# vlongle/pixie

Hardware: AMD Instinct MI355X
Metric: voxels/s (128^3 U-Net fwd) + MPM particle-steps/s (higher is better)
Workload: dtype f32 (operands split fp16 hi+lo, 3 f16 MFMAs/product, fp32 accumulate); 1 GPU; 128^3x64 feature grid -> SegmentationUNet+RegressionUNet forward (+argmax/one-hot combine), 1 scene per GPU per step; grid=128, feature_channels=64, parallelism=scene-parallel x1, executor=c+hip_graph

## Files before the change

### include/pixie_hip.h

```cpp
#ifndef PIXIE_HIP_H
#define PIXIE_HIP_H

#include <stdint.h>

#ifdef __cplusplus
extern "C" {
#endif

const char* pixie_last_error(void);
const char* pixie_build_arch(void);

typedef struct pixie_mpm pixie_mpm;

int pixie_mpm_create(pixie_mpm** out, int n_particles, int n_grid, double grid_lim);
int pixie_mpm_destroy(pixie_mpm* h);
int pixie_mpm_regrid(pixie_mpm* h, int n_grid, double grid_lim, void* stream);

int pixie_mpm_set_field(pixie_mpm* h, const char* name, const void* d_src, int64_t count, void* stream);
int pixie_mpm_get_field(pixie_mpm* h, const char* name, void* d_dst, int64_t count, void* stream);
int pixie_mpm_fill_field(pixie_mpm* h, const char* name, double value, void* stream);

int pixie_mpm_set_scalar(pixie_mpm* h, const char* key, double value);
int pixie_mpm_get_scalar(pixie_mpm* h, const char* key, double* value);

int pixie_mpm_update_mass(pixie_mpm* h, void* stream);
int pixie_mpm_finalize_mu_lam(pixie_mpm* h, int with_bulk, void* stream);
int pixie_mpm_apply_additional_params(pixie_mpm* h, const double point[3], const double size[3], double E,
                                      double nu, double density, int material, void* stream);
int pixie_mpm_apply_additional_params_batch(pixie_mpm* h, int64_t n_boxes, const float* d_boxes, const float* d_params,
                                            const int32_t* d_material, void* stream);

enum { PIXIE_BC_SURFACE = 0, PIXIE_BC_CUBOID = 1, PIXIE_BC_BBOX = 2 };
typedef struct pixie_bc_desc {
    int32_t type;
    int32_t surface_type;
    int32_t reset;
    int32_t pad_;
    double point[3], size[3], velocity[3], normal[3];
    double start_time, end_time, friction;
} pixie_bc_desc;
int pixie_mpm_add_bc(pixie_mpm* h, const pixie_bc_desc* bc);

enum { PIXIE_PM_IMPULSE = 0, PIXIE_PM_TRANSLATION = 1, PIXIE_PM_ROTATION = 2 };
typedef struct pixie_pmod_desc {
    int32_t type;
    int32_t pad_;
    double point[3], size[3];
    double force[3];
    double velocity[3];
    double normal[3], h1[3], h2[3];
    double half_height, radius, rotation_scale, translation_scale;
    double start_time, end_time;
} pixie_pmod_desc;
int pixie_mpm_add_particle_modifier(pixie_mpm* h, const pixie_pmod_desc* pm, void* stream);

int pixie_mpm_step(pixie_mpm* h, double dt, int n_substeps, void* stream);

typedef struct pixie_mpm_batch pixie_mpm_batch;
typedef struct pixie_batch_sched {
    double dt;
    int32_t steps_per_chunk;
    int32_t n_chunks;
    int32_t n_out;
    int32_t pad_;
    double shift[3], scale, mean[3];
    double inv_rotation[9];
    float* d_pos;
    float* d_cov;
} pixie_batch_sched;
int pixie_mpm_batch_create(pixie_mpm_batch** out, pixie_mpm* const* handles, int n_handles);
int pixie_mpm_batch_step(pixie_mpm_batch* b, double dt, int n_substeps, void* stream);
int pixie_mpm_batch_run(pixie_mpm_batch* b, const pixie_batch_sched* per_scene, int n_scenes, void* stream);
typedef struct pixie_batch_splat_out {
    float* d_log_scale;
    float* d_quat;
} pixie_batch_splat_out;
int pixie_mpm_batch_run_splats(pixie_mpm_batch* b, const pixie_batch_sched* per_scene, const pixie_batch_splat_out* splats ,
                               int n_scenes, void* stream);
int pixie_mpm_batch_destroy(pixie_mpm_batch* b);

int pixie_mpm_export_cov(pixie_mpm* h, float* d_cov , void* stream);
int pixie_mpm_export_R(pixie_mpm* h, float* d_R , void* stream);
int pixie_mpm_export_frame(pixie_mpm* h, int n_out, const double shift[3], double scale, const double mean[3],
                           const double inv_rotation[9], float* d_pos , float* d_cov ,
                           void* stream);
int pixie_splat_from_cov(const float* d_cov , int64_t n, float* d_log_scale , float* d_quat ,
                         void* stream);
int pixie_mpm_export_frame_splats(pixie_mpm* h, int n_out, const double shift[3], double scale, const double mean[3],
                                  const double inv_rotation[9], float* d_pos , float* d_cov ,
                                  float* d_log_scale , float* d_quat , void* stream);
int pixie_mpm_out_of_bounds(pixie_mpm* h, int64_t* count, void* stream);


typedef struct pixie_conv_desc {
    const float* d_in0; int32_t c0;
    const float* d_in1; int32_t c1;
    int32_t in_d, in_h, in_w;
    int32_t upsample;
    int32_t stride;
    int32_t ksize;
    const float* d_pro_a; const float* d_pro_b;
    const float* d_gamma; const float* d_beta;
    int32_t act;
    const float* d_w; const float* d_bias;
    int32_t c_out;
    const float* d_residual;
    float* d_out;
    const void* d_w16;
    const uint32_t* d_in_amax0; const uint32_t* d_in_amax1;
    float in_bound;
    float* d_out_stats;
    uint32_t* d_out_amax;
    void* d_workspace;
    int32_t out_d, out_h, out_w;
    const float* d_skip_in0; int32_t skip_c0;
    const float* d_skip_in1; int32_t skip_c1;
    const void* d_skip_w16; const float* d_skip_bias;
    const uint32_t* d_skip_amax0; const uint32_t* d_skip_amax1;
    int32_t w16_subpixel;
} pixie_conv_desc;

int pixie_conv_cout_padded(int c_out);
int pixie_conv_pack_weights(const float* d_w_oidhw, float* d_w_packed, int c_out, int c_in, int ksize, void* stream);
int64_t pixie_conv_packed16_bytes(int c_out, int c_in, int ksize);
int pixie_conv_pack_weights_f16x2(const float* d_w_oidhw, void* d_packed, int c_out, int c_in, int ksize, void* stream);
int64_t pixie_conv_subpixel_bytes(int c_out, int c_in);
int pixie_conv_pack_weights_subpixel(const float* d_w_oidhw, void* d_packed, int c_out, int c_in, void* stream);
int pixie_conv3d_forward(const pixie_conv_desc* desc, void* stream);
int64_t pixie_conv_stats_floats(const pixie_conv_desc* desc);
int64_t pixie_conv_workspace_bytes(const pixie_conv_desc* desc);
int pixie_stats_finalize(const float* d_stats, const pixie_conv_desc* desc, double* d_sums, void* stream);
int pixie_stats_norm_finalize(const float* d_stats0, const pixie_conv_desc* desc0, double* d_sums0, const float* d_stats1,
                              const pixie_conv_desc* desc1, double* d_sums1, int c1, int64_t spatial, int mode, int groups,
                              double eps, const float* d_weight, const float* d_bias, float* d_a, float* d_b, void* stream);
int pixie_conv_skip_foldable(const pixie_conv_desc* desc);

int pixie_channel_sums(const float* d_x, int channels, int64_t spatial, double* d_sums, void* stream);
int pixie_channel_stats(const float* d_x, int channels, int64_t spatial, double* d_sums, uint32_t* d_amax, void* stream);
int pixie_tensor_amax(const float* d_x, int64_t count, uint32_t* d_slot, void* stream);
int pixie_norm_finalize(const double* d_sums, int channels, int64_t spatial, int mode, int groups, double eps,
                        const float* d_weight, const float* d_bias, float* d_a, float* d_b, void* stream);

int pixie_attention_forward(const float* d_qkv, float* d_out, int channels, int tokens, void* stream);

int pixie_channel_affine(const float* d_x, const float* d_a, const float* d_b, float* d_y, int channels,
                         int64_t spatial, void* stream);

int pixie_voxel_grid_to_ncdhw(const void* d_feat_dhwc_f16, int d, int h, int w, int channels, float* d_out_cdhw, void* stream);

int pixie_projector_conv0(const void* d_feat_dhwc_f16, int64_t voxels, int channels, int n_networks, const void* const* d_w16,
                          const float* const* d_bias, float* const* d_out, int c_out, void* stream);

int pixie_pack_fields(const float* d_cont, const int32_t* d_seg_pred, int64_t n_scenes, int64_t spatial, void* d_wire, int64_t wire_bytes,
                      void* stream);

int pixie_combine_predictions(const float* d_logits, int num_classes, const float* d_cont, int64_t spatial,
                              float* d_combined, int32_t* d_argmax , void* stream);

int pixie_combine_class_ids(const int32_t* d_seg_pred, int num_classes, const float* d_cont, int64_t spatial, float* d_combined,
                            void* stream);

typedef struct pixie_unet pixie_unet;
typedef struct pixie_unet_config {
    int32_t feature_channels, cond_dim, model_channels, num_res_blocks;
    int32_t n_channel_mult; int32_t channel_mult[8];
    int32_t n_attention_resolutions; int32_t attention_resolutions[8];
    int32_t grid_size;
    int32_t out_channels;
    int32_t precision;
} pixie_unet_config;

int pixie_unet_create(pixie_unet** out, const pixie_unet_config* cfg);
int pixie_unet_destroy(pixie_unet* h);
int pixie_unet_param_count(const pixie_unet* h);
int pixie_unet_param_info(const pixie_unet* h, int index, const char** key, int64_t* numel, int32_t* ndim, int64_t shape[5]);
int pixie_unet_set_param(pixie_unet* h, const char* key, const float* d_values, int64_t numel);
int64_t pixie_unet_workspace_bytes(pixie_unet* h, int d, int hh, int w);
int pixie_unet_forward(pixie_unet* h, const float* d_feat, const float* d_proj0, int d, int hh, int w, float* d_out,
                       void* d_workspace, int64_t workspace_bytes, void* stream);
int pixie_unet_set_option(pixie_unet* h, const char* key, int value);

typedef struct pixie_field_desc {
    const float* d_pred;
    const uint8_t* d_mask;
    const float* d_axis_x; const float* d_axis_y; const float* d_axis_z;
    int32_t n_classes, d, h, w;
    double min_spacing;
    double density_min, density_max, E_min, E_max, nu_min, nu_max;
} pixie_field_desc;
int pixie_field_to_particles(const pixie_field_desc* field, const float* d_pos, int n, int k, double nn_distance_threshold,
                             int weighted, int default_material, int default_part_label, float* d_density, float* d_E,
                             float* d_nu, int32_t* d_material, int32_t* d_part_label, float* d_conf, float* d_nearest,
                             void* d_scratch, void* stream);

int pixie_unscale_prediction(const float* d_pred, int channels, int64_t spatial, double density_min, double density_max,
                             double E_min, double E_max, double nu_min, double nu_max, float* d_out, void* stream);
int64_t pixie_field_points_scratch_bytes(const pixie_field_desc* field);
int pixie_field_points(const pixie_field_desc* field, int64_t capacity, float* d_xyz , float* d_density, float* d_E,
                       float* d_nu, int32_t* d_material, float* d_conf, int64_t* d_count, void* d_scratch, void* stream);

int pixie_dbscan_roots(const float* d_pos_sorted, const int32_t* d_orig_index, const int32_t* d_cell_start, int n, int nx, int ny, int nz,
                       const double lo[3], double cell_size, double eps, int min_samples, int32_t* d_core_scratch,
                       int32_t* d_parent_scratch, int32_t* d_root, void* stream);

int pixie_fill_densify(const float* d_pos, const float* d_opacity, const float* d_cov6, int n, int grid_n, double grid_dx,
                       int32_t* d_grid_count, float* d_grid_density, void* stream);
int pixie_fill_dense_cells(int32_t* d_grid_count, const float* d_grid_density, int grid_n, double grid_dx, double density_thres,
                           int max_particles_per_cell, float* d_new_particles , int64_t max_samples,
                           uint64_t* d_counter, uint32_t seed, void* stream);
int pixie_fill_internal_cells(int32_t* d_grid_count, const float* d_grid_density, int grid_n, double grid_dx, int max_particles_per_cell,
                              int exclude_dir, int ray_cast_dir, double threshold, float* d_new_particles, int64_t max_samples,
                              uint64_t* d_counter, uint32_t seed, void* stream);
int pixie_particle_volume(const float* d_pos, int n, int grid_n, double grid_dx, int32_t* d_grid_count_scratch, float* d_vol, void* stream);
int pixie_nearest_particle(const float* d_pos, int n, const float* d_new_pos, int n_new, int32_t* d_nearest, void* stream);

typedef struct pixie_raster_desc {
    int32_t n, width, height;
    float tanfovx, tanfovy, scale_modifier;
    float viewmatrix[16], projmatrix[16], bg[3];
    int32_t pad_;
    const float* d_means;
    const float* d_cov3d;
    const float* d_scales;
    const float* d_rotations;
    const float* d_colors;
    const float* d_opacity;
    float* d_out_color;
    int32_t* d_radii;
    float* d_final_T;
    int32_t* d_n_contrib;
    void* d_workspace;
    int64_t workspace_bytes;
} pixie_raster_desc;
int64_t pixie_raster_workspace_bytes(int n, int width, int height, int64_t max_instances);
int pixie_raster_forward(const pixie_raster_desc* desc, int64_t* instances_out, void* stream);
int pixie_sh_to_rgb(const float* d_shs, int64_t n, int k_coeffs, int degree, const float* d_pos , const float campos[3],
                    const float* d_rot , int64_t n_rot, float* d_out , void* stream);

#ifdef PIXIE_DIAG
int pixie_mpm_phase(pixie_mpm* h, int phase, double dt, void* stream);

int pixie_mpm_kernel_times(pixie_mpm* h, double* particle_ms, double* grid_ms, int64_t* n_launches);

int pixie_conv_kernel_variant(const pixie_conv_desc* desc, int* slices);

int pixie_conv_tile_geometry(const pixie_conv_desc* desc, int32_t out[10]);
int pixie_conv_stats_layout(const pixie_conv_desc* desc, int64_t out[6]);
#endif

#ifdef __cplusplus
}
#endif
#endif
```

### pixie_amd/_lib.py

```python
from __future__ import annotations

import ctypes as C
import os

_HERE = os.path.dirname(os.path.abspath(__file__))
LIB_PATH = os.path.join(_HERE, "libpixie_hip.so")
DIAG_LIB_PATH = os.path.join(_HERE, "libpixie_hip_diag.so")


class PixieHipError(RuntimeError):
    pass


class BCDesc(C.Structure):
    _fields_ = [("type", C.c_int32), ("surface_type", C.c_int32), ("reset", C.c_int32), ("pad_", C.c_int32),
                ("point", C.c_double * 3), ("size", C.c_double * 3), ("velocity", C.c_double * 3),
                ("normal", C.c_double * 3), ("start_time", C.c_double), ("end_time", C.c_double),
                ("friction", C.c_double)]


class PModDesc(C.Structure):
    _fields_ = [("type", C.c_int32), ("pad_", C.c_int32),
                ("point", C.c_double * 3), ("size", C.c_double * 3), ("force", C.c_double * 3),
                ("velocity", C.c_double * 3), ("normal", C.c_double * 3), ("h1", C.c_double * 3),
                ("h2", C.c_double * 3), ("half_height", C.c_double), ("radius", C.c_double),
                ("rotation_scale", C.c_double), ("translation_scale", C.c_double),
                ("start_time", C.c_double), ("end_time", C.c_double)]


class ConvDesc(C.Structure):
    _fields_ = [("d_in0", C.c_void_p), ("c0", C.c_int32),
                ("d_in1", C.c_void_p), ("c1", C.c_int32),
                ("in_d", C.c_int32), ("in_h", C.c_int32), ("in_w", C.c_int32),
                ("upsample", C.c_int32), ("stride", C.c_int32), ("ksize", C.c_int32),
                ("d_pro_a", C.c_void_p), ("d_pro_b", C.c_void_p),
                ("d_gamma", C.c_void_p), ("d_beta", C.c_void_p),
                ("act", C.c_int32),
                ("d_w", C.c_void_p), ("d_bias", C.c_void_p),
                ("c_out", C.c_int32),
                ("d_residual", C.c_void_p), ("d_out", C.c_void_p),
                ("d_w16", C.c_void_p), ("d_in_amax0", C.c_void_p), ("d_in_amax1", C.c_void_p),
                ("in_bound", C.c_float),
                ("d_out_stats", C.c_void_p), ("d_out_amax", C.c_void_p),
                ("d_workspace", C.c_void_p),
                ("out_d", C.c_int32), ("out_h", C.c_int32), ("out_w", C.c_int32),
                ("d_skip_in0", C.c_void_p), ("skip_c0", C.c_int32),
                ("d_skip_in1", C.c_void_p), ("skip_c1", C.c_int32),
                ("d_skip_w16", C.c_void_p), ("d_skip_bias", C.c_void_p),
                ("d_skip_amax0", C.c_void_p), ("d_skip_amax1", C.c_void_p),
                ("w16_subpixel", C.c_int32)]


class UNetConfigC(C.Structure):
    _fields_ = [("feature_channels", C.c_int32), ("cond_dim", C.c_int32), ("model_channels", C.c_int32), ("num_res_blocks", C.c_int32),
                ("n_channel_mult", C.c_int32), ("channel_mult", C.c_int32 * 8),
                ("n_attention_resolutions", C.c_int32), ("attention_resolutions", C.c_int32 * 8),
                ("grid_size", C.c_int32), ("out_channels", C.c_int32), ("precision", C.c_int32)]


class BatchSched(C.Structure):
    _fields_ = [("dt", C.c_double), ("steps_per_chunk", C.c_int32), ("n_chunks", C.c_int32), ("n_out", C.c_int32), ("pad_", C.c_int32),
                ("shift", C.c_double * 3), ("scale", C.c_double), ("mean", C.c_double * 3), ("inv_rotation", C.c_double * 9),
                ("d_pos", C.c_void_p), ("d_cov", C.c_void_p)]


class BatchSplatOut(C.Structure):
    _fields_ = [("d_log_scale", C.c_void_p), ("d_quat", C.c_void_p)]


class FieldDesc(C.Structure):
    _fields_ = [("d_pred", C.c_void_p), ("d_mask", C.c_void_p),
                ("d_axis_x", C.c_void_p), ("d_axis_y", C.c_void_p), ("d_axis_z", C.c_void_p),
                ("n_classes", C.c_int32), ("d", C.c_int32), ("h", C.c_int32), ("w", C.c_int32),
                ("min_spacing", C.c_double),
                ("density_min", C.c_double), ("density_max", C.c_double), ("E_min", C.c_double), ("E_max", C.c_double),
                ("nu_min", C.c_double), ("nu_max", C.c_double)]


class RasterDesc(C.Structure):
    _fields_ = [("n", C.c_int32), ("width", C.c_int32), ("height", C.c_int32),
                ("tanfovx", C.c_float), ("tanfovy", C.c_float), ("scale_modifier", C.c_float),
                ("viewmatrix", C.c_float * 16), ("projmatrix", C.c_float * 16), ("bg", C.c_float * 3), ("pad_", C.c_int32),
                ("d_means", C.c_void_p), ("d_cov3d", C.c_void_p), ("d_scales", C.c_void_p), ("d_rotations", C.c_void_p),
                ("d_colors", C.c_void_p), ("d_opacity", C.c_void_p),
                ("d_out_color", C.c_void_p), ("d_radii", C.c_void_p), ("d_final_T", C.c_void_p), ("d_n_contrib", C.c_void_p),
                ("d_workspace", C.c_void_p), ("workspace_bytes", C.c_int64)]


_VP, _I, _I64, _D, _S = C.c_void_p, C.c_int, C.c_int64, C.c_double, C.c_char_p
_D3 = C.POINTER(C.c_double)
SIGNATURES = {
    "pixie_last_error": (C.c_char_p, []),
    "pixie_build_arch": (C.c_char_p, []),
    "pixie_mpm_create": (_I, [C.POINTER(_VP), _I, _I, _D]),
    "pixie_mpm_destroy": (_I, [_VP]),
    "pixie_mpm_regrid": (_I, [_VP, _I, _D, _VP]),
    "pixie_mpm_set_field": (_I, [_VP, _S, _VP, _I64, _VP]),
    "pixie_mpm_get_field": (_I, [_VP, _S, _VP, _I64, _VP]),
    "pixie_mpm_fill_field": (_I, [_VP, _S, _D, _VP]),
    "pixie_mpm_set_scalar": (_I, [_VP, _S, _D]),
    "pixie_mpm_get_scalar": (_I, [_VP, _S, C.POINTER(_D)]),
    "pixie_mpm_update_mass": (_I, [_VP, _VP]),
    "pixie_mpm_finalize_mu_lam": (_I, [_VP, _I, _VP]),
    "pixie_mpm_apply_additional_params": (_I, [_VP, _D3, _D3, _D, _D, _D, _I, _VP]),
    "pixie_mpm_apply_additional_params_batch": (_I, [_VP, _I64, _VP, _VP, _VP, _VP]),
    "pixie_mpm_add_bc": (_I, [_VP, C.POINTER(BCDesc)]),
    "pixie_mpm_add_particle_modifier": (_I, [_VP, C.POINTER(PModDesc), _VP]),
    "pixie_mpm_step": (_I, [_VP, _D, _I, _VP]),
    "pixie_mpm_export_cov": (_I, [_VP, _VP, _VP]),
    "pixie_mpm_export_R": (_I, [_VP, _VP, _VP]),
    "pixie_mpm_export_frame": (_I, [_VP, _I, _D3, _D, _D3, C.POINTER(C.c_double), _VP, _VP, _VP]),
    "pixie_mpm_out_of_bounds": (_I, [_VP, C.POINTER(_I64), _VP]),
    "pixie_mpm_batch_create": (_I, [C.POINTER(_VP), C.POINTER(_VP), _I]),
    "pixie_mpm_batch_step": (_I, [_VP, _D, _I, _VP]),
    "pixie_mpm_batch_run": (_I, [_VP, C.POINTER(BatchSched), _I, _VP]),
    "pixie_mpm_batch_run_splats": (_I, [_VP, C.POINTER(BatchSched), C.POINTER(BatchSplatOut), _I, _VP]),
    "pixie_splat_from_cov": (_I, [_VP, _I64, _VP, _VP, _VP]),
    "pixie_mpm_export_frame_splats": (_I, [_VP, _I, _D3, _D, _D3, C.POINTER(C.c_double), _VP, _VP, _VP, _VP, _VP]),
    "pixie_mpm_batch_destroy": (_I, [_VP]),
    "pixie_pack_fields": (_I, [_VP, _VP, _I64, _I64, _VP, _I64, _VP]),
    "pixie_conv_cout_padded": (_I, [_I]),
    "pixie_conv_pack_weights": (_I, [_VP, _VP, _I, _I, _I, _VP]),
    "pixie_conv_packed16_bytes": (_I64, [_I, _I, _I]),
    "pixie_conv_pack_weights_f16x2": (_I, [_VP, _VP, _I, _I, _I, _VP]),
    "pixie_conv_subpixel_bytes": (_I64, [_I, _I]),
    "pixie_conv_pack_weights_subpixel": (_I, [_VP, _VP, _I, _I, _VP]),
    "pixie_conv3d_forward": (_I, [C.POINTER(ConvDesc), _VP]),
    "pixie_conv_stats_floats": (_I64, [C.POINTER(ConvDesc)]),
    "pixie_conv_workspace_bytes": (_I64, [C.POINTER(ConvDesc)]),
    "pixie_stats_finalize": (_I, [_VP, C.POINTER(ConvDesc), _VP, _VP]),
    "pixie_stats_norm_finalize": (_I, [_VP, C.POINTER(ConvDesc), _VP, _VP, C.POINTER(ConvDesc), _VP, _I, _I64, _I, _I, _D, _VP, _VP, _VP, _VP, _VP]),
    "pixie_channel_stats": (_I, [_VP, _I, _I64, _VP, _VP, _VP]),
    "pixie_tensor_amax": (_I, [_VP, _I64, _VP, _VP]),
    "pixie_channel_sums": (_I, [_VP, _I, _I64, _VP, _VP]),
    "pixie_norm_finalize": (_I, [_VP, _I, _I64, _I, _I, _D, _VP, _VP, _VP, _VP, _VP]),
    "pixie_attention_forward": (_I, [_VP, _VP, _I, _I, _VP]),
    "pixie_channel_affine": (_I, [_VP, _VP, _VP, _VP, _I, _I64, _VP]),
    "pixie_projector_conv0": (_I, [_VP, _I64, _I, _I, C.POINTER(_VP), C.POINTER(_VP), C.POINTER(_VP), _I, _VP]),
    "pixie_conv_skip_foldable": (_I, [C.POINTER(ConvDesc)]),
    "pixie_unet_create": (_I, [C.POINTER(_VP), C.POINTER(UNetConfigC)]),
    "pixie_unet_destroy": (_I, [_VP]),
    "pixie_unet_param_count": (_I, [_VP]),
    "pixie_unet_param_info": (_I, [_VP, _I, C.POINTER(_S), C.POINTER(_I64), C.POINTER(C.c_int32), C.POINTER(_I64)]),
    "pixie_unet_set_param": (_I, [_VP, _S, _VP, _I64]),
    "pixie_unet_workspace_bytes": (_I64, [_VP, _I, _I, _I]),
    "pixie_unet_set_option": (_I, [_VP, _S, _I]),
    "pixie_unet_forward": (_I, [_VP, _VP, _VP, _I, _I, _I, _VP, _VP, _I64, _VP]),
    "pixie_combine_class_ids": (_I, [_VP, _I, _VP, _I64, _VP, _VP]),
    "pixie_combine_predictions": (_I, [_VP, _I, _VP, _I64, _VP, _VP, _VP]),
    "pixie_voxel_grid_to_ncdhw": (_I, [_VP, _I, _I, _I, _I, _VP, _VP]),
    "pixie_unscale_prediction": (_I, [_VP, _I, _I64, _D, _D, _D, _D, _D, _D, _VP, _VP]),
    "pixie_field_points_scratch_bytes": (_I64, [C.POINTER(FieldDesc)]),
    "pixie_field_points": (_I, [C.POINTER(FieldDesc), _I64, _VP, _VP, _VP, _VP, _VP, _VP, _VP, _VP, _VP]),
    "pixie_fill_densify": (_I, [_VP, _VP, _VP, _I, _I, _D, _VP, _VP, _VP]),
    "pixie_fill_dense_cells": (_I, [_VP, _VP, _I, _D, _D, _I, _VP, _I64, _VP, C.c_uint32, _VP]),
    "pixie_fill_internal_cells": (_I, [_VP, _VP, _I, _D, _I, _I, _I, _D, _VP, _I64, _VP, C.c_uint32, _VP]),
    "pixie_particle_volume": (_I, [_VP, _I, _I, _D, _VP, _VP, _VP]),
    "pixie_nearest_particle": (_I, [_VP, _I, _VP, _I, _VP, _VP]),
    "pixie_dbscan_roots": (_I, [_VP, _VP, _VP, _I, _I, _I, _I, C.POINTER(_D), _D, _D, _I, _VP, _VP, _VP, _VP]),
    "pixie_raster_workspace_bytes": (_I64, [_I, _I, _I, _I64]),
    "pixie_raster_forward": (_I, [C.POINTER(RasterDesc), C.POINTER(_I64), _VP]),
    "pixie_sh_to_rgb": (_I, [_VP, _I64, _I, _I, _VP, C.POINTER(C.c_float), _VP, _I64, _VP, _VP]),
    "pixie_field_to_particles": (_I, [C.POINTER(FieldDesc), _VP, _I, _I, _D, _I, _I, _I, _VP, _VP, _VP, _VP, _VP, _VP, _VP, _VP, _VP]),
}

DIAG_SIGNATURES = {
    "pixie_mpm_phase": (_I, [_VP, _I, _D, _VP]),
    "pixie_mpm_kernel_times": (_I, [_VP, C.POINTER(_D), C.POINTER(_D), C.POINTER(_I64)]),
    "pixie_conv_kernel_variant": (C.c_int, [C.POINTER(ConvDesc), C.POINTER(C.c_int)]),
    "pixie_conv_tile_geometry": (C.c_int, [C.POINTER(ConvDesc), C.POINTER(C.c_int32)]),
    "pixie_conv_stats_layout": (C.c_int, [C.POINTER(ConvDesc), C.POINTER(C.c_int64)]),
}

_libs = {}


def load(diag: bool = False):
    if diag in _libs:
        return _libs[diag]
    path = DIAG_LIB_PATH if diag else LIB_PATH
    if not os.path.exists(path):
        raise PixieHipError(
            f"{path} not found: build it with `python -m pixie_amd.build` (hipcc, gfx950). "
            "pixie_amd has no CPU fallback.")
    import torch
    lib = C.CDLL(path)
    for name, (res, args) in list(SIGNATURES.items()) + (list(DIAG_SIGNATURES.items()) if diag else []):
        fn = getattr(lib, name)
        fn.restype = res
        fn.argtypes = args
    _libs[diag] = lib
    return lib


def check(rc: int, what: str = "", lib=None):
    if rc != 0:
        msg = (lib or load()).pixie_last_error()
        raise PixieHipError(f"{what}: {msg.decode() if msg else 'unknown error'}")


def current_stream_ptr():
    import torch
    try:
        return C.c_void_p(torch._C._cuda_getCurrentRawStream(torch.cuda.current_device()))
    except AttributeError:
        return C.c_void_p(torch.cuda.current_stream().cuda_stream)


def d3(v):
    return (C.c_double * 3)(*[float(x) for x in v])
```

### pixie_amd/csrc/conv3d_f16x3.hip

```cpp
#include <hip/hip_runtime.h>

#include <cstdlib>
#include <map>
#include <string>
#include <type_traits>

#include "../../include/pixie_hip.h"
#include "common.h"
#include "conv_plan.h"

namespace pixie {

typedef float f32x16 __attribute__((ext_vector_type(16)));
typedef _Float16 f16x8 __attribute__((ext_vector_type(8)));

constexpr int kW16HeaderU4 = 4;

struct Conv16Args {
    const float* in0; const float* in1;
    int c0, cin;
    int ID, IH, IW;
    int LD, LH, LW;
    int ups;
    int stride;
// ... 786 lines not shown
    if (i < pairs)
        for (int pt = 0; pt < 64; ++pt) m = fmaxf(m, fabsf(subpixel_weight(src + i * 27, pt >> 3, pt & 7)));
    for (int off = 32; off > 0; off >>= 1) m = fmaxf(m, __shfl_down(m, off, 64));
    if ((threadIdx.x & 63) == 0 && m > 0.0f) atomicMax(slot, __float_as_uint(m));
}
__global__ void pack_weights_subpixel_kernel(const float* __restrict__ src, uint4* __restrict__ dst, int cout, int cin, int coutp,
                                             const unsigned* __restrict__ amax_bits) {
    const int KG = cin >> 3;
    const long total = 64L * KG * coutp;
    const long i = (long)blockIdx.x * blockDim.x + threadIdx.x;
    const int e = scale_exponent(__uint_as_float(*amax_bits));
    if (i == 0) dst[0] = make_uint4(__float_as_uint(pow2i(-e)), (unsigned)cout, (unsigned)cin, 64u);
    if (i >= total) return;
    const float s = pow2i(e);
    const int co = (int)(i % coutp);
    const long row = i / coutp;
    const int kg = (int)(row % KG);
    const int pt = (int)(row / KG);
    f16x8 vh, vl;
#pragma unroll
    for (int j = 0; j < 8; ++j) {
        float w = 0.0f;
        if (co < cout) w = subpixel_weight(src + ((long)co * cin + kg * 8 + j) * 27, pt >> 3, pt & 7) * s;
        const _Float16 h = (_Float16)w;
        vh[j] = h;
        vl[j] = (_Float16)(w - (float)h);
    }
    dst[kW16HeaderU4 + i] = __builtin_bit_cast(uint4, vh);
    dst[kW16HeaderU4 + total + i] = __builtin_bit_cast(uint4, vl);
}

static int reduce_segments(long osp) { return (int)((osp + kReduceSeg - 1) / kReduceSeg); }

bool conv_exact_v1() { return getenv("PIXIE_CONV_EXACT_V1") != nullptr; }

ConvShape conv_shape_of(const pixie_conv_desc* d) {
    ConvShape s;
    s.c0 = d->c0; s.c1 = d->c1; s.c_out = d->c_out;
    s.in_d = d->in_d; s.in_h = d->in_h; s.in_w = d->in_w;
    s.ksize = d->ksize; s.stride = d->stride; s.upsample = d->upsample;
    s.out_d = d->out_d; s.out_h = d->out_h; s.out_w = d->out_w;
    s.skip_c0 = d->skip_c0; s.skip_c1 = d->skip_c1;
    s.w16 = d->d_w16 != nullptr; s.subpixel = d->w16_subpixel != 0; s.workspace = d->d_workspace != nullptr; s.skip = d->d_skip_w16 != nullptr;
    s.exact_v1 = conv_exact_v1();
    return s;
}

static void conv_output_dims(const ConvShape& s, int& od, int& oh, int& ow) {
    const int pad = s.ksize == 3 ? 1 : 0;
    od = ((s.in_d << s.upsample) + 2 * pad - s.ksize) / s.stride + 1;
    oh = ((s.in_h << s.upsample) + 2 * pad - s.ksize) / s.stride + 1;
    ow = ((s.in_w << s.upsample) + 2 * pad - s.ksize) / s.stride + 1;
    if (s.out_d > 0) od = std::min(od, s.out_d);
    if (s.out_h > 0) oh = std::min(oh, s.out_h);
    if (s.out_w > 0) ow = std::min(ow, s.out_w);
}

ConvPlan conv_plan(const ConvShape& s) {
    ConvPlan p;
    auto refuse = [&p](ConvRefusal why) { p.path = CONV_NONE; p.refusal = why; return p; };
    if ((s.ksize != 1 && s.ksize != 3) || (s.stride != 1 && s.stride != 2) || (s.upsample != 0 && s.upsample != 1) || s.c0 <= 0 || s.c1 < 0 ||
        s.c_out <= 0 || s.in_d <= 0 || s.in_h <= 0 || s.in_w <= 0)
        return refuse(CONV_BAD_SHAPE);
    conv_output_dims(s, p.OD, p.OH, p.OW);
    p.KS = s.ksize; p.coutp = pixie_conv_cout_padded(s.c_out);
    p.ups = s.upsample; p.LD = s.in_d << p.ups; p.LH = s.in_h << p.ups; p.LW = s.in_w << p.ups;
    const int cin = s.c0 + s.c1;
    const bool stride_ok = s.stride == 1 || (s.ksize == 3 && !s.upsample), chunks_ok = cin % 16 == 0;
    if (!s.w16) {
        if (!stride_ok || !chunks_ok || s.exact_v1) { p.path = CONV_FIRST_GEN; return p; }
        p.path = CONV_EXACT_TILED;
    } else {
        if (!stride_ok) return refuse(CONV_BAD_STRIDE);
        if (!chunks_ok || s.c0 % 8 != 0) return refuse(CONV_BAD_CHANNELS);
        if (s.subpixel && !(s.upsample == 1 && s.ksize == 3 && s.stride == 1 && !s.skip)) return refuse(CONV_BAD_SUBPIXEL);
        p.path = s.subpixel ? CONV_F16X3_SUBPIXEL : CONV_F16X3;
    }
    const bool sub = p.path == CONV_F16X3_SUBPIXEL;
    const int chunks = cin / 16;
    const int smax = (p.f16x3() && s.workspace) ? std::min(8, chunks / 2) : 1;
    auto tile = [&p](int ED, int EH, int EW, int vox) {
        p.TX = pow2_le(EW, 32);
        p.TY = pow2_le(EH, std::max(1, std::min(4, vox / p.TX)));
        p.TZ = std::max(1, std::min(ED, vox / (p.TX * p.TY)));
        p.lTX = ilog2(p.TX); p.lTY = ilog2(p.TY);
        p.tiles_x = (EW + p.TX - 1) / p.TX; p.tiles_y = (EH + p.TY - 1) / p.TY; p.tiles_z = (ED + p.TZ - 1) / p.TZ;
        p.n_tiles = p.tiles_x * p.tiles_y * p.tiles_z;
    };
    if (sub) {
        p.ups = 0; p.LD = s.in_d; p.LH = s.in_h; p.LW = s.in_w;
        tile((p.OD + 1) / 2, (p.OH + 1) / 2, (p.OW + 1) / 2, 256);
        p.n_tiles *= 4;
        p.HX = p.TX + 2; p.HY = p.TY + 1; p.HZ = p.TZ + 1;
        p.MB = (p.coutp >= 64) ? 2 : 1; p.NB = 4;
        const long wgs = (long)p.n_tiles * ((p.coutp + p.MB * 32 - 1) / (p.MB * 32));
        while (p.slices * 2 <= smax && wgs * p.slices < 512) p.slices *= 2;
    } else {
        const long ovol = (long)p.OD * p.OH * p.OW;
        int MB = (p.coutp >= 64) ? 2 : 1;
        int NB = (s.stride == 2) ? 1 : 4;
        auto n_wg = [&](int mb, int nb) {
            const long tiles = (ovol + 128L * nb - 1) / (128L * nb);
            return tiles * ((p.coutp + mb * 32 - 1) / (mb * 32));
        };
        int slices = 1;
        if (smax >= 2 && n_wg(MB, NB) < 512) {
            bool found = false;
            for (int nb = NB; nb >= 1 && !found; nb /= 2) {
                for (int sl = 1; sl <= smax; sl *= 2)
                    if (n_wg(MB, nb) * sl >= 512) { NB = nb; slices = sl; found = true; break; }
            }
            if (!found) { NB = 1; slices = 1; while (slices * 2 <= smax) slices *= 2; }
        } else {
            while (n_wg(MB, NB) < 512 && NB > 1) NB /= 2;
            if (n_wg(MB, NB) < 512 && MB > 1) MB = 1;
        }
        p.MB = MB; p.NB = NB; p.slices = slices;
        tile(p.OD, p.OH, p.OW, 128 * NB);
        p.HX = (p.TX - 1) * s.stride + s.ksize; p.HY = (p.TY - 1) * s.stride + s.ksize; p.HZ = (p.TZ - 1) * s.stride + s.ksize;
    }
    p.HYX = p.HY * p.HX; p.CS = p.HZ * p.HYX;
    p.mHX = magic_of(p.HX); p.mHYX = magic_of(p.HYX);
    if (p.slices > 1) p.chunks_per_slice = (chunks + p.slices - 1) / p.slices;
    p.lds_bytes = (size_t)4 * p.CS * sizeof(uint4);
    if (p.lds_bytes > 160 * 1024) return refuse(CONV_BAD_LDS);
    const size_t epi_bytes = ((size_t)4 * 32 * (p.NB * 32 + 4) + (size_t)4 * p.MB * 32 * 2) * sizeof(float);
    if (p.slices == 1 && epi_bytes <= 80 * 1024) { p.epi_lds = 1; p.lds_bytes = std::max(p.lds_bytes, epi_bytes); }
    p.grid = dim3((unsigned)p.n_tiles, (unsigned)((p.coutp + p.MB * 32 - 1) / (p.MB * 32)), (unsigned)p.slices);
    if (!p.f16x3()) return p;
    const long osp = (long)p.OD * p.OH * p.OW;
    if (p.slices > 1) {
        const int n = reduce_segments(osp);
        p.stats = ConvStatLayout{n, n, 1, 1};
        p.stats_floats = (int64_t)s.c_out * n * 2 * (int64_t)(sizeof(double) / sizeof(float));
        p.workspace_bytes = (int64_t)p.slices * s.c_out * osp * (int64_t)sizeof(float);
    } else {
        p.stats = ConvStatLayout{p.n_tiles, 1, p.coutp, 0};
        p.stats_floats = (int64_t)p.n_tiles * p.coutp * 2;
    }
    p.fullres = !sub && p.slices == 1 && s.ksize == 3 && p.MB == 2 && p.NB == 4 && cin == 64 && s.c_out == 64 && s.stride == 1 && !s.upsample &&
                s.c1 == 0 && !s.skip && osp >= 128L * 128 * 128;
    const int scin = s.skip_c0 + s.skip_c1;
    p.skip_foldable = !sub && s.stride == 1 && !s.upsample && scin > 0 && scin % 16 == 0 && s.skip_c0 % 8 == 0 && p.slices == 1;
    return p;
}

using ConvKernel = void (*)(Conv16Args);
static ConvKernel conv16_kernel(const ConvPlan& p) {
    if (p.path == CONV_F16X3_SUBPIXEL) return p.MB == 2 ? conv3d_f16x3_subpixel_kernel<2> : conv3d_f16x3_subpixel_kernel<1>;
    if (p.fullres) return conv3d_f16x3_c64_fullres_kernel;
#define PX_CONV16_PICK(KS_, MB_, NB_) \
    if (p.KS == KS_ && p.MB == MB_ && p.NB == NB_) return p.path == CONV_EXACT_TILED ? conv3d_exact_kernel<KS_, MB_, NB_> : conv3d_f16x3_kernel<KS_, MB_, NB_>;
    PX_CONV_VARIANTS(PX_CONV16_PICK)
#undef PX_CONV16_PICK
    return nullptr;
}

static int launch(ConvKernel kern, const ConvPlan& p, const Conv16Args& a, hipStream_t st) {
    PX_REQUIRE(kern != nullptr, "conv: no kernel variant for ksize=%d MB=%d NB=%d", p.KS, p.MB, p.NB);
    PX_CHECK_HIP(allow_max_dynamic_lds(reinterpret_cast<const void*>(kern)));
    hipLaunchKernelGGL(kern, p.grid, dim3(256), p.lds_bytes, st, a);
    PX_CHECK_HIP(hipGetLastError());
    return 0;
}

static Conv16Args conv16_args(const pixie_conv_desc* d, const ConvPlan& p) {
    Conv16Args a{};
    a.in0 = d->d_in0; a.in1 = d->d_in1; a.c0 = d->c0; a.cin = d->c0 + d->c1;
    a.ID = d->in_d; a.IH = d->in_h; a.IW = d->in_w;
    a.LD = p.LD; a.LH = p.LH; a.LW = p.LW; a.ups = p.ups; a.stride = d->stride;
    a.OD = p.OD; a.OH = p.OH; a.OW = p.OW;
    a.pro_a = d->d_pro_a; a.pro_b = d->d_pro_b; a.gamma = d->d_gamma; a.beta = d->d_beta; a.act = d->act;
    a.bias = d->d_bias; a.cout = d->c_out; a.coutp = p.coutp;
    a.residual = d->d_residual; a.out = d->d_out;
    a.TX = p.TX; a.TY = p.TY; a.TZ = p.TZ; a.lTX = p.lTX; a.lTY = p.lTY;
    a.tiles_x = p.tiles_x; a.tiles_y = p.tiles_y; a.tiles_z = p.tiles_z; a.n_tiles = p.n_tiles;
    a.HX = p.HX; a.HY = p.HY; a.HZ = p.HZ; a.HYX = p.HYX; a.CS = p.CS; a.mHX = p.mHX; a.mHYX = p.mHYX;
    a.chunks_per_slice = p.chunks_per_slice; a.epi_lds = p.epi_lds;
    return a;
}

int conv3d_f16x3_forward(const pixie_conv_desc* d, const ConvPlan& p, hipStream_t st) {
    PX_REQUIRE(p.refusal != CONV_BAD_STRIDE, "f16x3 conv: stride must be 1, or 2 for a 3^3 kernel");
    PX_REQUIRE(p.refusal != CONV_BAD_CHANNELS, "f16x3 conv: c_in must be a multiple of 16 (got %d+%d)", d->c0, d->c1);
    PX_REQUIRE(d->d_in_amax0 != nullptr || d->in_bound > 0.0f, "f16x3 conv: needs d_in_amax0 or a positive in_bound");
    PX_REQUIRE(d->c1 == 0 || d->d_in_amax0 == nullptr || d->d_in_amax1 != nullptr, "f16x3 conv: second input needs its own amax slot");
    PX_REQUIRE(p.refusal != CONV_BAD_SUBPIXEL, "f16x3 conv: sub-pixel weights need upsample = 1, ksize = 3, stride = 1 and no folded skip");
    Conv16Args a = conv16_args(d, p);
    a.w16 = reinterpret_cast<const uint4*>(d->d_w16);
    a.amax0 = d->d_in_amax0; a.amax1 = (d->c1 > 0) ? d->d_in_amax1 : nullptr; a.in_bound = d->in_bound;
    a.stats = d->d_out_stats; a.out_amax = d->d_out_amax;
    if (d->d_skip_w16) {
        PX_REQUIRE(p.skip_foldable, "f16x3 conv: this launch cannot fold a skip convolution (pixie_conv_skip_foldable)");
        PX_REQUIRE(d->d_skip_in0 && d->d_skip_amax0 && (d->skip_c1 == 0 || (d->d_skip_in1 && d->d_skip_amax1)), "f16x3 conv: folded skip needs its inputs and their amax slots");
        a.sk_in0 = d->d_skip_in0; a.sk_in1 = d->d_skip_in1; a.sk_c0 = d->skip_c0; a.sk_cin = d->skip_c0 + d->skip_c1;
        a.sk_w16 = reinterpret_cast<const uint4*>(d->d_skip_w16); a.sk_bias = d->d_skip_bias;
        a.sk_amax0 = d->d_skip_amax0; a.sk_amax1 = d->skip_c1 > 0 ? d->d_skip_amax1 : nullptr;
    }
    if (p.slices > 1) {
        a.partial = static_cast<float*>(d->d_workspace);
        a.stats = nullptr; a.out_amax = nullptr;
    }
    PX_REQUIRE(p.refusal != CONV_BAD_LDS, "f16x3 conv: tile needs %zu B of LDS", p.lds_bytes);
    PX_REQUIRE(p.f16x3(), "f16x3 conv: bad sizes");
    if (int rc = launch(conv16_kernel(p), p, a, st)) return rc;
    if (p.slices == 1) return 0;
    const long osp = (long)a.OD * a.OH * a.OW, n_elems = (long)a.cout * osp;
    if (d->d_out_stats) {
        const dim3 rgrid((unsigned)reduce_segments(osp), (unsigned)a.cout);
        double* rstats = reinterpret_cast<double*>(d->d_out_stats);
        PX_REQUIRE((reinterpret_cast<size_t>(rstats) & 7) == 0, "f16x3 conv: d_out_stats of a split-K launch must be 8-byte aligned");
        const bool vec = osp % 4 == 0 && ((reinterpret_cast<size_t>(a.partial) | reinterpret_cast<size_t>(a.residual) | reinterpret_cast<size_t>(a.out)) & 15) == 0;
        if (vec) hipLaunchKernelGGL(splitk_reduce_stats_kernel<true>, rgrid, dim3(256), 0, st, a.partial, p.slices, n_elems, osp, a.bias, a.residual,
                                    a.out, rstats, d->d_out_amax);
        else hipLaunchKernelGGL(splitk_reduce_stats_kernel<false>, rgrid, dim3(256), 0, st, a.partial, p.slices, n_elems, osp, a.bias, a.residual,
                                a.out, rstats, d->d_out_amax);
    } else {
        hipLaunchKernelGGL(splitk_reduce_kernel, dim3((unsigned)((n_elems + 255) / 256)), dim3(256), 0, st, a.partial, p.slices, n_elems, osp,
                           a.bias, a.residual, a.out);
    }
    PX_CHECK_HIP(hipGetLastError());
    return 0;
}

int conv3d_exact_forward(const pixie_conv_desc* d, const ConvPlan& p, hipStream_t st) {
    PX_REQUIRE(p.refusal != CONV_BAD_LDS, "exact conv: tile needs %zu B of LDS", p.lds_bytes);
    PX_REQUIRE(p.path == CONV_EXACT_TILED, "exact conv: bad sizes");
    Conv16Args a = conv16_args(d, p);
    a.wf = d->d_w;
    a.in_bound = 1.0f;
    return launch(conv16_kernel(p), p, a, st);
}

}

using namespace pixie;

static ConvPlan plan_of(const pixie_conv_desc* d) { return d ? conv_plan(conv_shape_of(d)) : ConvPlan{}; }
static StatParts stat_parts(const ConvPlan& p, const void* stats) { return StatParts{stats, p.stats.n, p.stats.cstride, p.stats.tstride, p.stats.f64}; }

extern "C" int64_t pixie_conv_stats_floats(const pixie_conv_desc* d) { return plan_of(d).stats_floats; }

extern "C" int64_t pixie_conv_workspace_bytes(const pixie_conv_desc* d) {
    if (!d) return 0;
    ConvShape s = conv_shape_of(d);
    s.workspace = true;
    return conv_plan(s).workspace_bytes;
}

#ifdef PIXIE_DIAG
extern "C" int pixie_conv_kernel_variant(const pixie_conv_desc* d, int* slices_out) {
    const ConvPlan p = plan_of(d);
    if (slices_out) *slices_out = p.f16x3() ? p.slices : 1;
    if (!p.f16x3()) return 0;
    if (p.path == CONV_F16X3_SUBPIXEL) return 8300 + p.MB * 10 + p.NB;
    if (p.fullres) return 9324;
    return p.KS * 100 + p.MB * 10 + p.NB;
}

extern "C" int pixie_conv_tile_geometry(const pixie_conv_desc* d, int32_t out[10]) {
    const ConvPlan p = plan_of(d);
    if (!out || !p.tiled()) return 1;
    const int32_t v[10] = {p.TX, p.TY, p.TZ, p.tiles_x, p.tiles_y, p.tiles_z, p.epi_lds, p.slices, p.MB, p.NB};
    for (int i = 0; i < 10; ++i) out[i] = v[i];
    return 0;
}

extern "C" int pixie_conv_stats_layout(const pixie_conv_desc* d, int64_t out[6]) {
    const ConvPlan p = plan_of(d);
    if (!out || !p.f16x3()) return 1;
    out[0] = p.stats.n; out[1] = p.stats.cstride; out[2] = p.stats.tstride; out[3] = p.stats.f64; out[4] = p.stats.f64 ? kReduceSeg : 0;
    out[5] = p.coutp;
    return 0;
}
#endif

extern "C" int pixie_conv_skip_foldable(const pixie_conv_desc* d) { return plan_of(d).skip_foldable ? 1 : 0; }

extern "C" int pixie_stats_finalize(const float* d_stats, const pixie_conv_desc* d, double* d_sums, void* stream) {
    PX_REQUIRE(d_stats && d && d_sums, "pixie_stats_finalize: null argument");
    hipLaunchKernelGGL(stats_finalize_kernel, dim3((unsigned)d->c_out), dim3(256), 0, as_stream(stream), stat_parts(plan_of(d), d_stats), d_sums);
    PX_CHECK_HIP(hipGetLastError());
    return 0;
}

extern "C" int pixie_stats_norm_finalize(const float* d_stats0, const pixie_conv_desc* desc0, double* d_sums0, const float* d_stats1,
                                         const pixie_conv_desc* desc1, double* d_sums1, int c1, int64_t spatial, int mode, int groups,
                                         double eps, const float* d_weight, const float* d_bias, float* d_a, float* d_b, void* stream) {
    PX_REQUIRE(desc0 && d_sums0 && d_a && d_b && spatial > 0 && c1 >= 0, "pixie_stats_norm_finalize: bad arguments");
    PX_REQUIRE(c1 == 0 || d_sums1, "pixie_stats_norm_finalize: a second part needs d_sums1");
    PX_REQUIRE(!d_stats1 || desc1, "pixie_stats_norm_finalize: d_stats1 needs its descriptor");
    const int c0 = desc0->c_out, channels = c0 + c1;
    PX_REQUIRE(!d_stats1 || desc1->c_out == c1, "pixie_stats_norm_finalize: desc1 has %d output channels, c1 is %d", desc1 ? desc1->c_out : 0, c1);
    PX_REQUIRE(mode == 0 || (mode == 1 && groups > 0 && channels % groups == 0), "pixie_stats_norm_finalize: bad mode/groups");
    const StatParts none{nullptr, 0, 0, 0, 0};
    const StatParts p0 = d_stats0 ? stat_parts(plan_of(desc0), d_stats0) : none;
    const StatParts p1 = d_stats1 ? stat_parts(plan_of(desc1), d_stats1) : none;
    hipLaunchKernelGGL(stats_norm_finalize_kernel, dim3((unsigned)(mode == 0 ? channels : groups)), dim3(256), 0, as_stream(stream), p0, d_sums0, c0,
                       p1, d_sums1, channels, (double)spatial, mode, groups, eps, d_weight, d_bias, d_a, d_b);
    PX_CHECK_HIP(hipGetLastError());
    return 0;
}

extern "C" int64_t pixie_conv_packed16_bytes(int c_out, int c_in, int ksize) {
    if (c_out <= 0 || c_in <= 0 || c_in % 8 != 0 || (ksize != 1 && ksize != 3)) return 0;
    const int64_t taps = (int64_t)ksize * ksize * ksize;
    return ((int64_t)kW16HeaderU4 + 2 * taps * (c_in / 8) * pixie_conv_cout_padded(c_out)) * (int64_t)sizeof(uint4);
}

extern "C" int pixie_tensor_amax(const float* d_x, int64_t count, uint32_t* d_slot, void* stream) {
    PX_REQUIRE(d_x && d_slot && count > 0, "pixie_tensor_amax: bad arguments");
    const int blocks = (int)std::min<int64_t>(2048, (count + 1023) / 1024);
    hipLaunchKernelGGL(amax_kernel, dim3(blocks), dim3(256), 0, as_stream(stream), d_x, (long)count, d_slot);
    PX_CHECK_HIP(hipGetLastError());
    return 0;
}

extern "C" int pixie_conv_pack_weights_f16x2(const float* d_w, void* d_packed, int c_out, int c_in, int ksize, void* stream) {
    PX_REQUIRE(d_w && d_packed && c_out > 0 && c_in > 0 && c_in % 8 == 0 && (ksize == 1 || ksize == 3),
               "pixie_conv_pack_weights_f16x2: bad arguments (c_in must be a multiple of 8)");
    hipStream_t st = as_stream(stream);
    const int taps = ksize * ksize * ksize;
    const int coutp = pixie_conv_cout_padded(c_out);
    unsigned* slot = reinterpret_cast<unsigned*>(d_packed) + 15;
    PX_CHECK_HIP(hipMemsetAsync(d_packed, 0, kW16HeaderU4 * sizeof(uint4), st));
    if (pixie_tensor_amax(d_w, (int64_t)c_out * c_in * taps, slot, stream)) return 1;
    const long total = (long)taps * (c_in / 8) * coutp;
    hipLaunchKernelGGL(pack_weights_f16x2_kernel, dim3(cdiv(total, 256)), dim3(256), 0, st, d_w, reinterpret_cast<uint4*>(d_packed), c_out,
                       c_in, taps, coutp, slot);
    PX_CHECK_HIP(hipGetLastError());
    return 0;
}

extern "C" int64_t pixie_conv_subpixel_bytes(int c_out, int c_in) {
    if (c_out <= 0 || c_in <= 0 || c_in % 16 != 0) return 0;
    return ((int64_t)kW16HeaderU4 + 2 * 64 * (int64_t)(c_in / 8) * pixie_conv_cout_padded(c_out)) * (int64_t)sizeof(uint4);
}

extern "C" int pixie_conv_pack_weights_subpixel(const float* d_w, void* d_packed, int c_out, int c_in, void* stream) {
    PX_REQUIRE(d_w && d_packed && c_out > 0 && c_in > 0 && c_in % 16 == 0,
               "pixie_conv_pack_weights_subpixel: bad arguments (c_in must be a multiple of 16)");
    hipStream_t st = as_stream(stream);
    const int coutp = pixie_conv_cout_padded(c_out);
    unsigned* slot = reinterpret_cast<unsigned*>(d_packed) + 15;
    PX_CHECK_HIP(hipMemsetAsync(d_packed, 0, kW16HeaderU4 * sizeof(uint4), st));
    const long pairs = (long)c_out * c_in;
    hipLaunchKernelGGL(subpixel_amax_kernel, dim3(cdiv(pairs, 256)), dim3(256), 0, st, d_w, pairs, slot);
    PX_CHECK_HIP(hipGetLastError());
    const long total = 64L * (c_in / 8) * coutp;
    hipLaunchKernelGGL(pack_weights_subpixel_kernel, dim3(cdiv(total, 256)), dim3(256), 0, st, d_w, reinterpret_cast<uint4*>(d_packed), c_out,
                       c_in, coutp, slot);
    PX_CHECK_HIP(hipGetLastError());
    return 0;
}
```

### pixie_amd/csrc/projector_fused.hip

```cpp
#include <hip/hip_runtime.h>

#include "../../include/pixie_hip.h"
#include "common.h"

namespace pixie {

typedef float f32x16 __attribute__((ext_vector_type(16)));
typedef _Float16 f16x8 __attribute__((ext_vector_type(8)));

constexpr int kPW16HeaderU4 = 4;
constexpr int kPMaxNets = 2;
constexpr int kPKC = 64;

struct ProjArgs {
    const uint4* feat;
    long voxels;
    int C, KG;
    int nets, coutp, cout;
    const uint4* w16[kPMaxNets];
    const float* bias[kPMaxNets];
    float* out[kPMaxNets];
    int waves_m, nv;
};

__global__ __launch_bounds__(256, 2) void projector_conv0_kernel(ProjArgs A) {
    extern __shared__ uint4 xs[];
    const int tid = threadIdx.x, lane = tid & 63, wave = tid >> 6;
    const int kh = lane >> 5, l31 = lane & 31;
    const int wm = wave % A.waves_m, wn = wave / A.waves_m;
    const int row0 = wm * 64;
    const int net = row0 / A.coutp, co0 = row0 % A.coutp;
    const long v0 = (long)blockIdx.x * A.nv;
    const int vw = wn * 64;
    const int stride = A.nv + 1;

    f32x16 acc[2][2];
#pragma unroll
    for (int mb = 0; mb < 2; ++mb)
#pragma unroll
        for (int nb = 0; nb < 2; ++nb)
#pragma unroll
            for (int r = 0; r < 16; ++r) acc[mb][nb][r] = 0.0f;

    const uint4* wHi = A.w16[net] + kPW16HeaderU4 + co0 + l31;
    const size_t lo_off = (size_t)A.KG * A.coutp;
    const int units = A.nv * 8;

    for (int c_base = 0; c_base < A.C; c_base += kPKC) {
        __syncthreads();
        for (int u = tid; u < units; u += 256) {
            const int vox = u >> 3, kg = u & 7;
            const long v = v0 + vox;
            uint4 q = make_uint4(0u, 0u, 0u, 0u);
            if (v < A.voxels && c_base + 8 * kg < A.C) q = A.feat[v * A.KG + (c_base >> 3) + kg];
            xs[kg * stride + vox] = q;
        }
        __syncthreads();
#pragma unroll
        for (int ks = 0; ks < kPKC / 16; ++ks) {
            const int kg = (c_base >> 3) + 2 * ks + kh;
            if (c_base + 16 * ks >= A.C) break;
            f16x8 ah[2], al[2], b[2];
#pragma unroll
            for (int mb = 0; mb < 2; ++mb) {
                const uint4 h = wHi[(size_t)kg * A.coutp + mb * 32];
                const uint4 l = wHi[lo_off + (size_t)kg * A.coutp + mb * 32];
                ah[mb] = __builtin_bit_cast(f16x8, h);
                al[mb] = __builtin_bit_cast(f16x8, l);
            }
#pragma unroll
            for (int nb = 0; nb < 2; ++nb) b[nb] = __builtin_bit_cast(f16x8, xs[(2 * ks + kh) * stride + vw + nb * 32 + l31]);
#pragma unroll
            for (int mb = 0; mb < 2; ++mb)
#pragma unroll
                for (int nb = 0; nb < 2; ++nb) acc[mb][nb] = __builtin_amdgcn_mfma_f32_32x32x16_f16(al[mb], b[nb], acc[mb][nb], 0, 0, 0);
#pragma unroll
            for (int mb = 0; mb < 2; ++mb)
#pragma unroll
                for (int nb = 0; nb < 2; ++nb) acc[mb][nb] = __builtin_amdgcn_mfma_f32_32x32x16_f16(ah[mb], b[nb], acc[mb][nb], 0, 0, 0);
        }
    }

    const float inv = __uint_as_float(A.w16[net][0].x);
    float* out = A.out[net];
    const float* bias = A.bias[net];
#pragma unroll
    for (int mb = 0; mb < 2; ++mb)
#pragma unroll
        for (int r = 0; r < 16; ++r) {
            const int co = co0 + mb * 32 + (r & 3) + 8 * (r >> 2) + 4 * kh;
            if (co >= A.cout) continue;
            const float bv = bias ? bias[co] : 0.0f;
#pragma unroll
            for (int nb = 0; nb < 2; ++nb) {
                const long v = v0 + vw + nb * 32 + l31;
                if (v < A.voxels) out[(size_t)co * A.voxels + v] = acc[mb][nb][r] * inv + bv;
            }
        }
}

}

using namespace pixie;

extern "C" int pixie_projector_conv0(const void* d_feat_dhwc_f16, int64_t voxels, int channels, int n_networks, const void* const* d_w16,
                                     const float* const* d_bias, float* const* d_out, int c_out, void* stream) {
    PX_REQUIRE(d_feat_dhwc_f16 && d_w16 && d_out && voxels > 0, "pixie_projector_conv0: null argument");
    PX_REQUIRE(n_networks >= 1 && n_networks <= kPMaxNets, "pixie_projector_conv0: 1 or 2 networks");
    PX_REQUIRE(channels > 0 && channels % 16 == 0, "pixie_projector_conv0: the channel count must be a multiple of 16 (got %d)", channels);
    const int coutp = pixie_conv_cout_padded(c_out);
    PX_REQUIRE(c_out > 0 && coutp % 64 == 0, "pixie_projector_conv0: c_out must pad to a multiple of 64 (got %d -> %d)", c_out, coutp);
    const int rows = n_networks * coutp;
    PX_REQUIRE(rows == 64 || rows == 128 || rows == 256, "pixie_projector_conv0: %d x %d output rows are not a tiling this kernel has", n_networks, coutp);
    ProjArgs a{};
    a.feat = static_cast<const uint4*>(d_feat_dhwc_f16);
    a.voxels = voxels; a.C = channels; a.KG = channels / 8;
    a.nets = n_networks; a.coutp = coutp; a.cout = c_out;
    for (int n = 0; n < n_networks; ++n) {
        PX_REQUIRE(d_w16[n] && d_out[n], "pixie_projector_conv0: null weights / output for network %d", n);
        a.w16[n] = static_cast<const uint4*>(d_w16[n]);
        a.bias[n] = d_bias ? d_bias[n] : nullptr;
        a.out[n] = d_out[n];
    }
    a.waves_m = rows / 64;
    a.nv = (4 / a.waves_m) * 64;
    const size_t lds = (size_t)8 * (a.nv + 1) * sizeof(uint4);
    const long tiles = (voxels + a.nv - 1) / a.nv;
    hipLaunchKernelGGL(projector_conv0_kernel, dim3((unsigned)tiles), dim3(256), lds, as_stream(stream), a);
    PX_CHECK_HIP(hipGetLastError());
    return 0;
}
```

### pixie_amd/csrc/unet_exec.hip

```cpp
#include <hip/hip_runtime.h>

#include <algorithm>
#include <cmath>
#include <cstdlib>
#include <cstring>
#include <map>
#include <memory>
#include <stdexcept>
#include <string>
#include <tuple>
#include <unordered_map>
#include <vector>

#include "../../include/pixie_hip.h"
#include "common.h"
#include "conv_plan.h"

namespace pixie {
int channel_stats_prezeroed(const float* d_x, int channels, int64_t spatial, double* d_sums, uint32_t* d_amax, hipStream_t st);
int norm_finalize_cat(const double* d_sums0, int c0, const double* d_sums1, int c1, int64_t spatial, int mode, int groups, double eps,
                      const float* d_weight, const float* d_bias, float* d_a, float* d_b, hipStream_t st);
namespace {

enum { ACT_NONE = 0, ACT_LEAKY = 1, ACT_SILU = 2 };
enum Kind { CONV_IN, RES, DOWN, ATTN, UP };

struct Blk { Kind kind; std::string prefix; int cin, cout, sp; };
struct Plan {
    std::vector<std::vector<Blk>> in_blocks, out_blocks;
    std::vector<Blk> middle;
    int out_sp = 0;
};

struct Err : std::runtime_error { using std::runtime_error::runtime_error; };
[[noreturn]] void fail(const char* fmt, ...) {
    char buf[512];
    va_list ap; va_start(ap, fmt); vsnprintf(buf, sizeof buf, fmt, ap); va_end(ap);
    throw Err(buf);
}
void ok(int rc, const char* what) { if (rc != 0) fail("%s: %s", what, pixie_last_error()); }

bool has(const std::vector<int>& v, int x) { for (int e : v) if (e == x) return true; return false; }

struct Cfg {
    int feature_channels, cond_dim, model_channels, num_res_blocks;
    std::vector<int> mult, attn;
    int grid_size, out_channels, precision;
    bool has_projector() const { return feature_channels != cond_dim; }
    int projector_hidden() const { return feature_channels > cond_dim ? 128 : 0; }
};

Plan build_plan(const Cfg& c) {
    Plan p;
    const int mc = c.model_channels, nrb = c.num_res_blocks;
    auto name = [](const char* part, int idx, int sub) { return std::string("unet.") + part + "." + std::to_string(idx) + "." + std::to_string(sub); };
    p.in_blocks.push_back({Blk{CONV_IN, "unet.input_blocks.0.0", c.cond_dim, mc, c.grid_size}});
    std::vector<int> chans{mc}, sizes{c.grid_size};
    int ch = mc, ds = 1, sp = c.grid_size;
    for (size_t level = 0; level < c.mult.size(); ++level) {
        const int m = c.mult[level];
        for (int r = 0; r < nrb; ++r) {
            const int idx = (int)p.in_blocks.size();
            std::vector<Blk> seq{Blk{RES, name("input_blocks", idx, 0), ch, m * mc, sp}};
            ch = m * mc;
            if (has(c.attn, ds)) seq.push_back(Blk{ATTN, name("input_blocks", idx, 1), ch, ch, sp});
            p.in_blocks.push_back(seq);
            chans.push_back(ch);
        }
        if (level + 1 != c.mult.size()) {
            const int idx = (int)p.in_blocks.size();
            p.in_blocks.push_back({Blk{DOWN, name("input_blocks", idx, 0), ch, ch, sp}});
            chans.push_back(ch);
            sizes.push_back(sp);
            ds *= 2;
            sp = (sp + 1) / 2;
        }
    }
    p.middle = {Blk{RES, "unet.middle_block.0", ch, ch, sp}, Blk{ATTN, "unet.middle_block.1", ch, ch, sp}, Blk{RES, "unet.middle_block.2", ch, ch, sp}};
    for (int level = (int)c.mult.size() - 1; level >= 0; --level) {
        const int m = c.mult[level];
        for (int i = 0; i <= nrb; ++i) {
            const int idx = (int)p.out_blocks.size();
            const int ich = chans.back(); chans.pop_back();
            std::vector<Blk> seq{Blk{RES, name("output_blocks", idx, 0), ch + ich, mc * m, sp}};
            ch = mc * m;
            if (has(c.attn, ds)) seq.push_back(Blk{ATTN, name("output_blocks", idx, (int)seq.size()), ch, ch, sp});
            if (level && i == nrb) {
                seq.push_back(Blk{UP, name("output_blocks", idx, (int)seq.size()), ch, ch, sp});
                ds /= 2;
                sp = sizes.back(); sizes.pop_back();
            }
            p.out_blocks.push_back(seq);
        }
    }
    p.out_sp = sp;
    return p;
}

struct Param {
    std::string key;
    std::vector<int64_t> shape;
    int64_t numel = 1;
    bool norm = false;
    const float* d = nullptr;
    uint64_t version = 0;
};

std::vector<Param> param_table(const Cfg& c, const Plan& plan) {
    std::vector<Param> out;
    auto add = [&](const std::string& key, std::vector<int64_t> shape, bool norm) {
        Param p; p.key = key; p.shape = shape; p.norm = norm;
        for (int64_t s : shape) p.numel *= s;
        out.push_back(p);
    };
    auto conv = [&](const std::string& prefix, int cout, int cin, int k, int dims = 3) {
        std::vector<int64_t> s{cout, cin};
        for (int i = 0; i < dims; ++i) s.push_back(k);
        add(prefix + ".weight", s, false);
        add(prefix + ".bias", {cout}, false);
    };
    auto norm = [&](const std::string& prefix, std::vector<int64_t> shape) {
        add(prefix + ".weight", shape, true);
        add(prefix + ".bias", shape, true);
    };
    if (c.has_projector()) {
        const int hid = c.projector_hidden();
        if (!hid) {
            conv("projector.net.0", c.cond_dim, c.feature_channels, 1);
            norm("projector.net.1", {c.cond_dim});
        } else {
            conv("projector.net.0", hid, c.feature_channels, 1);
            norm("projector.net.1", {hid});
            conv("projector.net.3", hid, hid, 3);
            norm("projector.net.4", {hid});
            conv("projector.net.6", c.cond_dim, hid, 1);
            norm("projector.net.7", {c.cond_dim});
        }
    }
    auto emit = [&](const Blk& b) {
        const std::vector<int64_t> vol{b.sp, b.sp, b.sp};
        switch (b.kind) {
            case CONV_IN: conv(b.prefix, b.cout, b.cin, 3); break;
            case RES:
                norm(b.prefix + ".in_layers.0", vol);
                conv(b.prefix + ".in_layers.2", b.cout, b.cin, 3);
                norm(b.prefix + ".out_layers.0", vol);
                conv(b.prefix + ".out_layers.3", b.cout, b.cout, 3);
                if (b.cin != b.cout) conv(b.prefix + ".skip_connection", b.cout, b.cin, 1);
                break;
            case DOWN: conv(b.prefix + ".op", b.cout, b.cin, 3); break;
            case UP:   conv(b.prefix + ".conv", b.cout, b.cin, 3); break;
            case ATTN:
                norm(b.prefix + ".norm", {b.cin});
                conv(b.prefix + ".qkv", 3 * b.cin, b.cin, 1, 1);
                conv(b.prefix + ".proj_out", b.cin, b.cin, 1, 1);
                break;
        }
    };
    for (auto& seq : plan.in_blocks) for (auto& b : seq) emit(b);
    for (auto& b : plan.middle) emit(b);
    for (auto& seq : plan.out_blocks) for (auto& b : seq) emit(b);
    norm("unet.out.0", {plan.out_sp, plan.out_sp, plan.out_sp});
    conv("unet.out.2", c.out_channels, c.model_channels, 3);
    return out;
}

struct Arena {
    static constexpr int64_t kAlign = 256;
    char* base = nullptr;
    int64_t capacity = 0, peak = 0;
    std::map<int64_t, int64_t> free_;
    std::map<int64_t, int64_t> used_;

    void reset(char* b, int64_t cap) {
        base = b; capacity = cap; peak = 0;
        free_.clear(); used_.clear();
        free_[0] = cap;
    }
    int64_t alloc(int64_t bytes) {
        bytes = (bytes + kAlign - 1) / kAlign * kAlign;
        if (bytes == 0) bytes = kAlign;
        for (auto it = free_.begin(); it != free_.end(); ++it) {
            if (it->second < bytes) continue;
            const int64_t off = it->first, rest = it->second - bytes;
            free_.erase(it);
            if (rest > 0) free_[off + bytes] = rest;
            used_[off] = bytes;
            if (off + bytes > peak) peak = off + bytes;
            return off;
        }
        fail("pixie_unet_forward: the workspace is too small (%lld bytes; ask pixie_unet_workspace_bytes for this grid size)", (long long)capacity);
    }
    void release(int64_t off) {
        auto u = used_.find(off);
        if (u == used_.end()) return;
        int64_t size = u->second;
        used_.erase(u);
        auto next = free_.lower_bound(off);
        if (next != free_.end() && off + size == next->first) { size += next->second; next = free_.erase(next); }
        if (next != free_.begin()) {
            auto prev = std::prev(next);
            if (prev->first + prev->second == off) { prev->second += size; return; }
        }
        free_[off] = size;
    }
    template <class T> T* ptr(int64_t off) const { return reinterpret_cast<T*>(base + off); }
};

struct Exec;
struct Tens {
    Exec* ex = nullptr;
    float* p = nullptr;
    int64_t off = -1;
    int c = 0, d = 0, h = 0, w = 0;
    int64_t sums_off = -1;
    bool has_sums = false;
    double* sums = nullptr;
    int64_t partials_off = -1;
    pixie_conv_desc pdesc;
    uint32_t* slot = nullptr;
    int64_t spatial() const { return (int64_t)d * h * w; }
    ~Tens();
};
using TP = std::shared_ptr<Tens>;

struct Packed { void* d = nullptr; uint64_t version = ~0ull; };
struct Sized { int64_t bytes; int slots; int64_t zsum_doubles; };
struct Bound { float wmax = 0, bmax = 0; uint64_t wver = ~0ull, bver = ~0ull; };

}
}

using namespace pixie;

struct pixie_unet {
    Cfg cfg;
    Plan plan;
    std::vector<Param> params;
    std::unordered_map<std::string, int> index;
    std::unordered_map<std::string, Packed> packed32, packed16;
    std::unordered_map<std::string, Bound> bounds;
    uint32_t* d_bound_slots = nullptr;
    std::vector<uint32_t> h_bound_slots;
    std::map<std::tuple<int, int, int, bool>, Sized> sized;
    bool fuse_stats = true, split_k = true, fold_skip = true, subpixel = true;
    bool split_stats = true;
    struct Replay { const float* feat; const float* proj0; float* out; void* ws; int d; uint64_t epoch; hipGraph_t graph; hipGraphExec_t exec; };
    bool use_graph = false;
    uint64_t epoch = 0;
    std::vector<Replay> replays;
    static constexpr size_t kMaxReplays = 4;
    void drop_replay(size_t i) {
        (void)hipGraphExecDestroy(replays[i].exec);
        (void)hipGraphDestroy(replays[i].graph);
        replays.erase(replays.begin() + (long)i);
    }

    const Param& param(const std::string& key) const {
        auto it = index.find(key);
        if (it == index.end()) fail("pixie_unet: no parameter named '%s'", key.c_str());
        return params[it->second];
    }
};

namespace pixie {
namespace {

struct Exec {
    pixie_unet* net = nullptr;
    Arena arena;
    bool dry = false;
    void* stream = nullptr;
    uint32_t* slots = nullptr;
    int slot_next = 0, slot_cap = 0;
    double* zsums = nullptr;
    int64_t zsum_next = 0, zsum_cap = 0;

    TP make(int c, int d, int h, int w) {
        auto t = std::make_shared<Tens>();
        t->ex = this; t->c = c; t->d = d; t->h = h; t->w = w;
        t->off = arena.alloc((int64_t)c * d * h * w * sizeof(float));
        t->p = arena.ptr<float>(t->off);
        return t;
    }
    TP external(const float* p, int c, int d, int h, int w) {
        auto t = std::make_shared<Tens>();
        t->ex = this; t->p = const_cast<float*>(p); t->c = c; t->d = d; t->h = h; t->w = w;
        return t;
    }
    uint32_t* new_slot() {
        if (!dry && slot_next >= slot_cap) fail("pixie_unet_forward: out of |x|max slots (internal sizing error)");
        return dry ? (slot_next++, nullptr) : slots + slot_next++;
    }
    struct Scratch {
        Exec* ex; int64_t off;
        Scratch(Exec* e, int64_t bytes) : ex(e), off(e->arena.alloc(bytes)) {}
        ~Scratch() { ex->arena.release(off); }
        template <class T> T* as() const { return ex->arena.ptr<T>(off); }
    };

    const float* P(const std::string& key) {
        const Param& p = net->param(key);
        if (!dry && !p.d) fail("pixie_unet_forward: parameter '%s' was never set", key.c_str());
        return p.d;
    }
    const void* w16(const std::string& key, bool subpixel = false) {
        const Param& p = net->param(key + ".weight");
        if (dry) return nullptr;
        Packed& e = net->packed16[subpixel ? key + "#subpixel" : key];
        if (e.version != p.version) {
            const int cout = (int)p.shape[0], cin = (int)p.shape[1], k = (int)p.shape[2];
            const int64_t nb = subpixel ? (k == 3 ? pixie_conv_subpixel_bytes(cout, cin) : 0) : pixie_conv_packed16_bytes(cout, cin, k);
            if (nb <= 0) fail("pixie_unet: '%s' cannot take the f16x3 packing (c_in %d)", key.c_str(), cin);
            if (!e.d && hipMalloc(&e.d, (size_t)nb) != hipSuccess) fail("pixie_unet: hipMalloc of %lld bytes failed", (long long)nb);
            if (!p.d) fail("pixie_unet_forward: parameter '%s.weight' was never set", key.c_str());
            if (subpixel) ok(pixie_conv_pack_weights_subpixel(p.d, e.d, cout, cin, stream), "pixie_conv_pack_weights_subpixel");
            else ok(pixie_conv_pack_weights_f16x2(p.d, e.d, cout, cin, k, stream), "pixie_conv_pack_weights_f16x2");
            e.version = p.version;
        }
        return e.d;
    }
    const float* w32(const std::string& key) {
        const Param& p = net->param(key + ".weight");
        if (dry) return nullptr;
        Packed& e = net->packed32[key];
        if (e.version != p.version) {
            const int cout = (int)p.shape[0], cin = (int)p.shape[1], k = (int)p.shape[2];
            int64_t taps = 1;
            for (size_t i = 2; i < p.shape.size(); ++i) taps *= p.shape[i];
            const int64_t nb = taps * cin * pixie_conv_cout_padded(cout) * (int64_t)sizeof(float);
            if (!e.d && hipMalloc(&e.d, (size_t)nb) != hipSuccess) fail("pixie_unet: hipMalloc of %lld bytes failed", (long long)nb);
            if (!p.d) fail("pixie_unet_forward: parameter '%s.weight' was never set", key.c_str());
            ok(pixie_conv_pack_weights(p.d, static_cast<float*>(e.d), cout, cin, k, stream), "pixie_conv_pack_weights");
            e.version = p.version;
        }
        return static_cast<const float*>(e.d);
    }
    float norm_bound(const std::string& key, int64_t count) {
        if (dry) return 1.0f;
        const Bound& b = net->bounds[key];
        return (float)(std::sqrt((double)count) * (double)b.wmax + (double)b.bmax + 1e-30);
    }

    void stats(const TP& t) {
        if (t->has_sums || t->partials_off >= 0) return;
        t->has_sums = true;
        if (!dry && zsum_next + 2 * t->c > zsum_cap) fail("pixie_unet_forward: out of statistics space (internal sizing error)");
        t->sums = dry ? nullptr : zsums + zsum_next;
        zsum_next += 2 * t->c;
        t->slot = new_slot();
        if (!dry) ok(channel_stats_prezeroed(t->p, t->c, t->spatial(), t->sums, t->slot, as_stream(stream)), "pixie_channel_stats");
    }
    struct AB { std::shared_ptr<Scratch> mem; float* a; float* b; };
    AB norm_finalize(const std::vector<TP>& parts, int64_t spatial, int mode, int groups, const float* w, const float* b) {
        for (auto& t : parts) stats(t);
        const Tens* t0 = parts[0].get();
        const Tens* t1 = parts.size() > 1 ? parts[1].get() : nullptr;
        const int c0 = t0->c, c1 = t1 ? t1->c : 0, c = c0 + c1;
        AB r;
        const int cpad = (c + 63) / 64 * 64;
        r.mem = std::make_shared<Scratch>(this, (int64_t)(cpad + c) * sizeof(float));
        r.a = r.mem->as<float>();
        r.b = r.a + cpad;
        const bool p0 = t0->partials_off >= 0, p1 = t1 && t1->partials_off >= 0;
        if (p0 || p1) {
            pixie_conv_desc d0 = t0->pdesc;
            if (!p0) { std::memset(&d0, 0, sizeof d0); d0.c_out = c0; }
            if (!dry) ok(pixie_stats_norm_finalize(p0 ? arena.ptr<float>(t0->partials_off) : nullptr, &d0, t0->sums,
                                                   p1 ? arena.ptr<float>(t1->partials_off) : nullptr, p1 ? &t1->pdesc : nullptr, t1 ? t1->sums : nullptr,
                                                   c1, spatial, mode, groups, 1e-5, w, b, r.a, r.b, stream), "pixie_stats_norm_finalize");
            for (auto& t : parts)
                if (t->partials_off >= 0) { arena.release(t->partials_off); t->partials_off = -1; t->has_sums = true; }
        } else if (!t1) {
            if (!dry) ok(pixie_norm_finalize(t0->sums, c, spatial, mode, groups, 1e-5, w, b, r.a, r.b, stream), "pixie_norm_finalize");
        } else {
            if (!dry) ok(norm_finalize_cat(t0->sums, c0, t1->sums, c1, spatial, mode, groups, 1e-5, w, b, r.a, r.b, as_stream(stream)), "pixie_norm_finalize");
        }
        return r;
    }

    ConvPlan plan_conv(ConvShape& s, const std::vector<TP>& parts, int cout, int ksize, int stride, bool upsample) const {
        s.c0 = parts[0]->c; s.c1 = parts.size() > 1 ? parts[1]->c : 0; s.c_out = cout;
        s.in_d = parts[0]->d; s.in_h = parts[0]->h; s.in_w = parts[0]->w;
        s.ksize = ksize; s.stride = stride; s.upsample = upsample ? 1 : 0;
        s.w16 = net->cfg.precision == 0; s.workspace = net->split_k; s.exact_v1 = conv_exact_v1();
        ConvPlan p = conv_plan(s);
        if (p.refusal == CONV_BAD_CHANNELS) { s.w16 = s.subpixel = s.skip = false; p = conv_plan(s); }
        return p;
    }
    bool skip_foldable(const TP& x, int cout, int ksize, const std::vector<TP>& sp) const {
        ConvShape s;
        s.skip_c0 = sp[0]->c; s.skip_c1 = sp.size() > 1 ? sp[1]->c : 0;
        return plan_conv(s, {x}, cout, ksize, 1, false).skip_foldable;
    }

    struct ConvOpt {
        int stride = 1; bool upsample = false;
        const AB* pro = nullptr; std::string affine_store;
        int act = ACT_NONE; TP residual; float bound = 0.0f;
        int out_d = 0, out_h = 0, out_w = 0;
        float* out_ptr = nullptr;
        const std::vector<TP>* skip_parts = nullptr; std::string skip_key;
    };
    TP conv(const std::vector<TP>& parts, const std::string& wkey, int cout, int ksize, const ConvOpt& o) {
        const TP& x0 = parts[0];
        const Tens* x1 = parts.size() > 1 ? parts[1].get() : nullptr;
        ConvShape s;
        s.out_d = o.out_d; s.out_h = o.out_h; s.out_w = o.out_w;
        s.subpixel = net->subpixel && o.upsample && ksize == 3 && o.stride == 1;
        if (o.skip_parts) { s.skip = true; s.skip_c0 = (*o.skip_parts)[0]->c; s.skip_c1 = o.skip_parts->size() > 1 ? (*o.skip_parts)[1]->c : 0; }
        const ConvPlan plan = plan_conv(s, parts, cout, ksize, o.stride, o.upsample);
        const int od = plan.OD, oh = plan.OH, ow = plan.OW;
        pixie_conv_desc desc;
        std::memset(&desc, 0, sizeof desc);
        if (o.out_d) { desc.out_d = od; desc.out_h = oh; desc.out_w = ow; }
        const bool f16 = s.w16;
        const bool raw = !o.pro && o.affine_store.empty();
        if (f16 && raw) for (auto& t : parts) stats(t);

        TP out = o.out_ptr ? external(o.out_ptr, cout, od, oh, ow) : make(cout, od, oh, ow);
        desc.d_in0 = x0->p; desc.c0 = x0->c;
        desc.d_in1 = x1 ? x1->p : nullptr; desc.c1 = x1 ? x1->c : 0;
        desc.in_d = x0->d; desc.in_h = x0->h; desc.in_w = x0->w;
        desc.upsample = o.upsample ? 1 : 0;
        desc.stride = o.stride;
        desc.ksize = ksize;
        if (o.pro) { desc.d_pro_a = o.pro->a; desc.d_pro_b = o.pro->b; }
        if (!o.affine_store.empty()) { desc.d_gamma = P(o.affine_store + ".weight"); desc.d_beta = P(o.affine_store + ".bias"); }
        desc.act = o.act;
        desc.d_bias = P(wkey + ".bias");
        desc.c_out = cout;
        desc.d_residual = o.residual ? o.residual->p : nullptr;
        desc.d_out = out->p;
        if (!f16) {
            desc.d_w = w32(wkey);
            if (!dry) ok(pixie_conv3d_forward(&desc, stream), "pixie_conv3d_forward");
            return out;
        }
        desc.d_w16 = w16(wkey, s.subpixel);
        desc.w16_subpixel = s.subpixel ? 1 : 0;
        if (o.skip_parts) {
            const std::vector<TP>& sp = *o.skip_parts;
            desc.d_skip_in0 = sp[0]->p; desc.skip_c0 = sp[0]->c;
            desc.d_skip_in1 = sp.size() > 1 ? sp[1]->p : nullptr; desc.skip_c1 = sp.size() > 1 ? sp[1]->c : 0;
            desc.d_skip_w16 = w16(o.skip_key);
            desc.d_skip_bias = P(o.skip_key + ".bias");
            desc.d_skip_amax0 = sp[0]->slot; desc.d_skip_amax1 = sp.size() > 1 ? sp[1]->slot : nullptr;
        }
        if (raw) {
            desc.d_in_amax0 = parts[0]->slot;
            desc.d_in_amax1 = x1 ? parts[1]->slot : nullptr;
        } else {
            desc.in_bound = o.bound;
        }
        std::unique_ptr<Scratch> workspace;
        if (plan.workspace_bytes > 0) { workspace.reset(new Scratch(this, plan.workspace_bytes)); desc.d_workspace = workspace->as<void>(); }
        bool have_stats = false;
        if (net->fuse_stats) {
            uint32_t* slot = new_slot();
            const int64_t nfl = plan.stats_floats;
            if (nfl > 0 && (!workspace || net->split_stats)) {
                out->partials_off = arena.alloc(nfl * (int64_t)sizeof(float));
                desc.d_out_stats = arena.ptr<float>(out->partials_off);
                desc.d_out_amax = slot;
                have_stats = true;
                out->slot = slot;
            }
        }
        if (!dry) ok(pixie_conv3d_forward(&desc, stream), "pixie_conv3d_forward");
        if (have_stats) {
            out->sums_off = arena.alloc((int64_t)cout * 2 * sizeof(double));
            out->sums = arena.ptr<double>(out->sums_off);
            out->pdesc = desc;
        }
        return out;
    }

    TP res(const Blk& b, const std::vector<TP>& parts) {
        const std::string& p = b.prefix;
        const int64_t spatial = parts[0]->spatial();
        AB pro = norm_finalize(parts, spatial, 0, 1, nullptr, nullptr);
        ConvOpt o1; o1.pro = &pro; o1.affine_store = p + ".in_layers.0"; o1.act = ACT_LEAKY; o1.bound = norm_bound(p + ".in_layers.0", spatial);
        TP h = conv(parts, p + ".in_layers.2", b.cout, 3, o1);
        AB pro2 = norm_finalize({h}, spatial, 0, 1, nullptr, nullptr);
        TP skip = parts[0];
        ConvOpt o2; o2.pro = &pro2; o2.affine_store = p + ".out_layers.0"; o2.act = ACT_LEAKY; o2.bound = norm_bound(p + ".out_layers.0", spatial);
        if (b.cin != b.cout) {
            if (net->fold_skip && skip_foldable(h, b.cout, 3, parts)) {
                skip.reset();
                for (auto& t : parts) stats(t);
                o2.skip_parts = &parts; o2.skip_key = p + ".skip_connection";
            } else {
                skip = conv(parts, p + ".skip_connection", b.cout, 1, ConvOpt{});
            }
        }
        o2.residual = skip;
        return conv({h}, p + ".out_layers.3", b.cout, 3, o2);
    }
    TP attn(const Blk& b, const TP& x) {
        const std::string& p = b.prefix;
        const int c = x->c;
        const int64_t spatial = x->spatial();
        AB pro = norm_finalize({x}, spatial, 1, 32, P(p + ".norm.weight"), P(p + ".norm.bias"));
        ConvOpt o; o.pro = &pro; o.bound = norm_bound(p + ".norm", spatial * (c / 32));
        TP qkv = conv({x}, p + ".qkv", 3 * c, 1, o);
        TP att = make(c, x->d, x->h, x->w);
        if (!dry) ok(pixie_attention_forward(qkv->p, att->p, c, (int)spatial, stream), "pixie_attention_forward");
        qkv.reset();
        ConvOpt o2; o2.residual = x;
        return conv({att}, p + ".proj_out", c, 1, o2);
    }
    TP block(const Blk& b, const std::vector<TP>& parts, const Tens* up_to) {
        if (b.kind == RES) return res(b, parts);
        const TP& x = parts[0];
        if (b.kind == ATTN) return attn(b, x);
        if (b.kind == DOWN) { ConvOpt o; o.stride = 2; return conv({x}, b.prefix + ".op", b.cout, 3, o); }
        if (b.kind == UP) {
            ConvOpt o; o.upsample = true;
            if (up_to) { o.out_d = up_to->d; o.out_h = up_to->h; o.out_w = up_to->w; }
            return conv({x}, b.prefix + ".conv", b.cout, 3, o);
        }
        fail("pixie_unet: unexpected block kind");
    }

    TP forward(const float* d_feat, const float* d_proj0, int D, int H, int W, float* d_out) {
        const Cfg& c = net->cfg;
        const int64_t spatial = (int64_t)D * H * W;
        TP x;
        AB pro_in; const AB* pro_in_p = nullptr;
        int act_in = ACT_NONE; float bound_in = 0.0f;
        if (c.has_projector()) {
            const std::string q = "projector.net.";
            const int hid = c.projector_hidden();
            if (!hid) {
                const int g = std::max(c.cond_dim / 2, 1);
                x = conv({external(d_feat, c.feature_channels, D, H, W)}, q + "0", c.cond_dim, 1, ConvOpt{});
                pro_in = norm_finalize({x}, spatial, 1, g, P(q + "1.weight"), P(q + "1.bias"));
                act_in = ACT_SILU;
                bound_in = norm_bound(q + "1", spatial * (c.cond_dim / g));
            } else {
                if (d_proj0) x = external(d_proj0, hid, D, H, W);
                else x = conv({external(d_feat, c.feature_channels, D, H, W)}, q + "0", hid, 1, ConvOpt{});
                AB pro = norm_finalize({x}, spatial, 1, 32, P(q + "1.weight"), P(q + "1.bias"));
                ConvOpt o; o.pro = &pro; o.act = ACT_SILU; o.bound = norm_bound(q + "1", spatial * (hid / 32));
                x = conv({x}, q + "3", hid, 3, o);
                AB pro2 = norm_finalize({x}, spatial, 1, 32, P(q + "4.weight"), P(q + "4.bias"));
                ConvOpt o2; o2.pro = &pro2; o2.act = ACT_SILU; o2.bound = norm_bound(q + "4", spatial * (hid / 32));
                x = conv({x}, q + "6", c.cond_dim, 1, o2);
                pro_in = norm_finalize({x}, spatial, 1, 32, P(q + "7.weight"), P(q + "7.bias"));
                bound_in = norm_bound(q + "7", spatial * std::max(c.cond_dim / 32, 1));
            }
            pro_in_p = &pro_in;
        } else {
            x = external(d_feat, c.feature_channels, D, H, W);
        }
        const Plan& plan = net->plan;
        std::vector<TP> hs;
        const Blk& first = plan.in_blocks[0][0];
        ConvOpt of; of.pro = pro_in_p; of.act = act_in; of.bound = bound_in;
        TP h = conv({x}, first.prefix, first.cout, 3, of);
        x.reset();
        pro_in = AB{};
        hs.push_back(h);
        for (size_t i = 1; i < plan.in_blocks.size(); ++i) {
            for (const Blk& b : plan.in_blocks[i]) h = block(b, {h}, nullptr);
            hs.push_back(h);
        }
        for (const Blk& b : plan.middle) h = block(b, {h}, nullptr);
        for (auto& seq : plan.out_blocks) {
            TP skip = hs.back(); hs.pop_back();
            if (skip->d != h->d || skip->h != h->h || skip->w != h->w) fail("pixie_unet_forward: skip tensor and decoder tensor differ in size");
            std::vector<TP> parts{h, skip};
            h.reset(); skip.reset();
            for (const Blk& b : seq) {
                TP nh = block(b, parts, (b.kind == UP && !hs.empty()) ? hs.back().get() : nullptr);
                parts.clear();
                parts.push_back(nh);
            }
            h = parts[0];
        }
        AB pro = norm_finalize({h}, h->spatial(), 0, 1, nullptr, nullptr);
        ConvOpt oo; oo.pro = &pro; oo.affine_store = "unet.out.0"; oo.act = ACT_LEAKY; oo.bound = norm_bound("unet.out.0", h->spatial());
        oo.out_ptr = d_out;
        return conv({h}, "unet.out.2", c.out_channels, 3, oo);
    }
};

Tens::~Tens() {
    if (!ex) return;
    if (off >= 0) ex->arena.release(off);
    if (sums_off >= 0) ex->arena.release(sums_off);
    if (partials_off >= 0) ex->arena.release(partials_off);
}

void refresh_bounds(pixie_unet* net, void* stream) {
    std::vector<std::pair<std::string, int>> todo;
    int n_norm = 0;
    for (const Param& p : net->params) {
        if (!p.norm || p.key.size() < 7 || p.key.compare(p.key.size() - 7, 7, ".weight") != 0) continue;
        const std::string key = p.key.substr(0, p.key.size() - 7);
        const Param& pb = net->param(key + ".bias");
        Bound& b = net->bounds[key];
        if (b.wver != p.version || b.bver != pb.version) todo.push_back({key, 2 * n_norm});
        ++n_norm;
    }
    if (todo.empty()) return;
    const size_t bytes = (size_t)2 * n_norm * sizeof(uint32_t);
    if (!net->d_bound_slots && hipMalloc(&net->d_bound_slots, bytes) != hipSuccess) fail("pixie_unet: hipMalloc failed");
    net->h_bound_slots.assign((size_t)2 * n_norm, 0u);
    hipStream_t s = as_stream(stream);
    if (hipMemsetAsync(net->d_bound_slots, 0, bytes, s) != hipSuccess) fail("pixie_unet: hipMemsetAsync failed");
    for (auto& t : todo) {
        const Param& pw = net->param(t.first + ".weight");
        const Param& pb = net->param(t.first + ".bias");
        if (!pw.d || !pb.d) fail("pixie_unet_forward: parameter '%s' was never set", t.first.c_str());
        ok(pixie_tensor_amax(pw.d, pw.numel, net->d_bound_slots + t.second, stream), "pixie_tensor_amax");
        ok(pixie_tensor_amax(pb.d, pb.numel, net->d_bound_slots + t.second + 1, stream), "pixie_tensor_amax");
    }
    if (hipMemcpyAsync(net->h_bound_slots.data(), net->d_bound_slots, bytes, hipMemcpyDeviceToHost, s) != hipSuccess ||
        hipStreamSynchronize(s) != hipSuccess)
        fail("pixie_unet: reading the normalisation bounds back failed: %s", hipGetErrorString(hipGetLastError()));
    for (auto& t : todo) {
        Bound& b = net->bounds[t.first];
        std::memcpy(&b.wmax, &net->h_bound_slots[t.second], 4);
        std::memcpy(&b.bmax, &net->h_bound_slots[t.second + 1], 4);
        b.wver = net->param(t.first + ".weight").version;
        b.bver = net->param(t.first + ".bias").version;
    }
}

__global__ void zero_head_kernel(uint4* p, int64_t n16) {
    const int64_t i = (int64_t)blockIdx.x * 256 + threadIdx.x;
    if (i < n16) p[i] = make_uint4(0u, 0u, 0u, 0u);
}

constexpr int64_t kSlotAlign = 256;
int64_t slot_region_bytes(int n_slots) { return ((int64_t)n_slots * 4 + kSlotAlign - 1) / kSlotAlign * kSlotAlign; }
int64_t zsum_region_bytes(int64_t n_doubles) { return (n_doubles * 8 + kSlotAlign - 1) / kSlotAlign * kSlotAlign; }

Sized size_pass(pixie_unet* net, int D, int H, int W, bool from_proj0) {
    auto key = std::make_tuple(D, H, W, from_proj0);
    auto it = net->sized.find(key);
    if (it != net->sized.end()) return it->second;
    Exec ex;
    ex.net = net; ex.dry = true; ex.stream = nullptr;
    ex.arena.reset(reinterpret_cast<char*>(0x10000000), (int64_t)1 << 50);
    {
        const float* fake = reinterpret_cast<const float*>(0x100);
        TP out = ex.forward(from_proj0 ? nullptr : fake, from_proj0 ? fake : nullptr, D, H, W, reinterpret_cast<float*>(0x100));
    }
    Sized r{ex.arena.peak + slot_region_bytes(ex.slot_next) + zsum_region_bytes(ex.zsum_next), ex.slot_next, ex.zsum_next};
    net->sized[key] = r;
    return r;
}

template <class F> int guarded(F f) {
    try { return f(); }
    catch (const std::exception& e) { return set_error("%s", e.what()); }
}

}
}

extern "C" int pixie_unet_create(pixie_unet** out, const pixie_unet_config* c) {
    PX_REQUIRE(out && c, "pixie_unet_create: null argument");
    PX_REQUIRE(c->n_channel_mult >= 1 && c->n_channel_mult <= 8 && c->n_attention_resolutions >= 0 && c->n_attention_resolutions <= 8,
               "pixie_unet_create: channel_mult needs 1..8 entries, attention_resolutions 0..8");
    PX_REQUIRE(c->feature_channels > 0 && c->cond_dim > 0 && c->model_channels > 0 && c->num_res_blocks > 0 && c->grid_size > 0 && c->out_channels > 0,
               "pixie_unet_create: non-positive size");
    PX_REQUIRE(c->precision == 0 || c->precision == 1, "pixie_unet_create: precision is 0 (f16x3) or 1 (exact fp32)");
    return guarded([&] {
        std::unique_ptr<pixie_unet> n(new pixie_unet);
        n->cfg.feature_channels = c->feature_channels; n->cfg.cond_dim = c->cond_dim; n->cfg.model_channels = c->model_channels;
        n->cfg.num_res_blocks = c->num_res_blocks; n->cfg.grid_size = c->grid_size; n->cfg.out_channels = c->out_channels;
        n->cfg.precision = c->precision;
        n->cfg.mult.assign(c->channel_mult, c->channel_mult + c->n_channel_mult);
        n->cfg.attn.assign(c->attention_resolutions, c->attention_resolutions + c->n_attention_resolutions);
        n->plan = build_plan(n->cfg);
        n->params = param_table(n->cfg, n->plan);
        for (size_t i = 0; i < n->params.size(); ++i) n->index[n->params[i].key] = (int)i;
        const char* fs = getenv("PIXIE_FUSE_STATS"); n->fuse_stats = !(fs && fs[0] == '0');
        const char* sk = getenv("PIXIE_CONV_SPLIT_K"); n->split_k = !(sk && sk[0] == '0');
        const char* fk = getenv("PIXIE_FOLD_SKIP"); n->fold_skip = !(fk && fk[0] == '0');
        const char* ss = getenv("PIXIE_SPLIT_STATS"); n->split_stats = !(ss && ss[0] == '0');
        const char* sx = getenv("PIXIE_CONV_SUBPIXEL"); n->subpixel = !(sx && sx[0] == '0');
        *out = n.release();
        return 0;
    });
}

extern "C" int pixie_unet_destroy(pixie_unet* h) {
    if (!h) return 0;
    for (auto& kv : h->packed16) if (kv.second.d) (void)hipFree(kv.second.d);
    for (auto& kv : h->packed32) if (kv.second.d) (void)hipFree(kv.second.d);
    if (h->d_bound_slots) (void)hipFree(h->d_bound_slots);
    while (!h->replays.empty()) h->drop_replay(0);
    delete h;
    return 0;
}

extern "C" int pixie_unet_param_count(const pixie_unet* h) { return h ? (int)h->params.size() : 0; }

extern "C" int pixie_unet_param_info(const pixie_unet* h, int i, const char** key, int64_t* numel, int32_t* ndim, int64_t shape[5]) {
    PX_REQUIRE(h && i >= 0 && i < (int)h->params.size(), "pixie_unet_param_info: index out of range");
    const Param& p = h->params[i];
    if (key) *key = p.key.c_str();
    if (numel) *numel = p.numel;
    if (ndim) *ndim = (int32_t)p.shape.size();
    if (shape) for (size_t k = 0; k < p.shape.size() && k < 5; ++k) shape[k] = p.shape[k];
    return 0;
}

extern "C" int pixie_unet_set_param(pixie_unet* h, const char* key, const float* d_values, int64_t numel) {
    PX_REQUIRE(h && key && d_values, "pixie_unet_set_param: null argument");
    auto it = h->index.find(key);
    PX_REQUIRE(it != h->index.end(), "pixie_unet_set_param: unexpected key '%s' (the reference's load_state_dict(strict=True) raises here too)", key);
    Param& p = h->params[it->second];
    PX_REQUIRE(numel == p.numel, "pixie_unet_set_param: '%s' has %lld elements, got %lld", key, (long long)p.numel, (long long)numel);
    p.d = d_values;
    ++p.version;
    ++h->epoch;
    return 0;
}

extern "C" int64_t pixie_unet_workspace_bytes(pixie_unet* h, int d, int hh, int w) {
    if (!h || d <= 0 || hh <= 0 || w <= 0) { set_error("pixie_unet_workspace_bytes: bad argument"); return -1; }
    int64_t bytes = -1;
    const int rc = guarded([&] {
        bytes = size_pass(h, d, hh, w, false).bytes;
        if (h->cfg.projector_hidden() > 0) bytes = std::max(bytes, size_pass(h, d, hh, w, true).bytes);
        return 0;
    });
    return rc == 0 ? bytes : -1;
}

extern "C" int pixie_unet_forward(pixie_unet* h, const float* d_feat, const float* d_proj0, int d, int hh, int w, float* d_out,
                                  void* d_workspace, int64_t workspace_bytes, void* stream) {
    PX_REQUIRE(h && d_out && d_workspace && (d_feat || d_proj0), "pixie_unet_forward: null argument");
    PX_REQUIRE(d == h->cfg.grid_size && hh == d && w == d,
               "pixie_unet_forward: the network was built for a %d^3 grid (its LayerNorm parameters have that shape), got %d x %d x %d", h->cfg.grid_size, d, hh, w);
    PX_REQUIRE(!d_proj0 || h->cfg.projector_hidden() > 0, "pixie_unet_forward: d_proj0 needs the hidden-128 projector (feature_channels > cond_dim)");
    PX_REQUIRE(d_feat || (d_proj0 && h->cfg.has_projector()), "pixie_unet_forward: d_feat is null");
    return guarded([&] {
        const auto sized = size_pass(h, d, hh, w, d_proj0 != nullptr);
        if (workspace_bytes < sized.bytes)
            fail("pixie_unet_forward: workspace of %lld bytes, this grid needs %lld (pixie_unet_workspace_bytes)", (long long)workspace_bytes, (long long)sized.bytes);
        auto launch_all = [&] {
            Exec ex;
            ex.net = h; ex.dry = false; ex.stream = stream;
            const int64_t slot_bytes = slot_region_bytes(sized.slots), head_bytes = slot_bytes + zsum_region_bytes(sized.zsum_doubles);
            ex.slots = static_cast<uint32_t*>(d_workspace);
            ex.slot_cap = sized.slots;
            ex.zsums = reinterpret_cast<double*>(static_cast<char*>(d_workspace) + slot_bytes);
            ex.zsum_cap = sized.zsum_doubles;
            hipLaunchKernelGGL(zero_head_kernel, dim3((unsigned)((head_bytes / 16 + 255) / 256)), dim3(256), 0, as_stream(stream),
                               static_cast<uint4*>(d_workspace), head_bytes / 16);
            if (hipGetLastError() != hipSuccess) fail("pixie_unet_forward: clearing the workspace head failed");
            ex.arena.reset(static_cast<char*>(d_workspace) + head_bytes, workspace_bytes - head_bytes);
            TP out = ex.forward(d_feat, d_proj0, d, hh, w, d_out);
        };
        if (h->use_graph) {
            for (size_t i = 0; i < h->replays.size(); ++i) {
                const pixie_unet::Replay& r = h->replays[i];
                if (r.feat != d_feat || r.proj0 != d_proj0 || r.out != d_out || r.ws != d_workspace || r.d != d) continue;
                if (r.epoch != h->epoch) { h->drop_replay(i); break; }
                if (hipGraphLaunch(r.exec, as_stream(stream)) != hipSuccess) fail("pixie_unet_forward: hipGraphLaunch failed: %s", hipGetErrorString(hipGetLastError()));
                if (i + 1 != h->replays.size()) std::rotate(h->replays.begin() + (long)i, h->replays.begin() + (long)i + 1, h->replays.end());
                return 0;
            }
        }
        if (h->use_graph && as_stream(stream) == nullptr)
            fail("pixie_unet_forward: option \"graph\" needs a non-default stream (the legacy stream cannot be captured); pass a created stream or set graph = 0");
        refresh_bounds(h, stream);
        launch_all();
        if (h->use_graph) {
            hipStream_t st = as_stream(stream);
            if (hipStreamBeginCapture(st, hipStreamCaptureModeThreadLocal) != hipSuccess)
                fail("pixie_unet_forward: cannot capture on this stream (graph replay needs a non-default stream): %s", hipGetErrorString(hipGetLastError()));
            hipGraph_t graph = nullptr;
            try { launch_all(); }
            catch (...) { (void)hipStreamEndCapture(st, &graph); if (graph) (void)hipGraphDestroy(graph); throw; }
            if (hipStreamEndCapture(st, &graph) != hipSuccess || !graph) fail("pixie_unet_forward: hipStreamEndCapture failed: %s", hipGetErrorString(hipGetLastError()));
            hipGraphExec_t exec = nullptr;
            if (hipGraphInstantiate(&exec, graph, nullptr, nullptr, 0) != hipSuccess) { (void)hipGraphDestroy(graph); fail("pixie_unet_forward: hipGraphInstantiate failed"); }
            if (h->replays.size() >= pixie_unet::kMaxReplays) h->drop_replay(0);
            h->replays.push_back(pixie_unet::Replay{d_feat, d_proj0, d_out, d_workspace, d, h->epoch, graph, exec});
        }
        return 0;
    });
}

extern "C" int pixie_unet_set_option(pixie_unet* h, const char* key, int value) {
    PX_REQUIRE(h && key, "pixie_unet_set_option: null argument");
    const std::string k(key);
    if (k == "graph") {
        h->use_graph = value != 0;
        if (!h->use_graph) while (!h->replays.empty()) h->drop_replay(0);
        return 0;
    }
    return set_error("pixie_unet_set_option: unknown key '%s' (known: graph)", key);
}
```

### pixie_amd/unet.py

```python
from __future__ import annotations

import ctypes as C
import math
import os
import warnings
import weakref
from typing import Dict, List, Optional, Sequence, Tuple

import torch
import torch.nn as nn

from . import _lib
from ._lib import ConvDesc, check
from .unet_plan import Block, UNetConfig, UNetPlan, build_plan, param_shapes, is_norm_key

ACT_NONE, ACT_LEAKY, ACT_SILU = 0, 1, 2
DEFAULT_PRECISION = os.environ.get("PIXIE_CONV_PRECISION", "f16x3")
_ZERO_INIT_SUFFIXES = (".out_layers.3.weight", ".out_layers.3.bias", ".proj_out.weight", ".proj_out.bias",
                       "unet.out.2.weight", "unet.out.2.bias")


def _ptr(t: Optional[torch.Tensor]):
    return C.c_void_p(t.data_ptr()) if t is not None else C.c_void_p(0)


def _addr(t: Optional[torch.Tensor]):
    return t.data_ptr() if t is not None else None


def fill_conv_desc(lib, alloc, parts: Sequence[torch.Tensor], packed_w, bias, cout: int, ksize: int, *, stride: int = 1,
                   upsample: bool = False, pro=None, affine=None, act: int = 0, residual=None, w16=None, in_amax=None,
                   in_bound: float = 0.0, out_amax=None, out_size=None, skip=None, subpixel: bool = False, split_k: bool = True,
                   split_stats: bool = False, addr=_addr):
    x0 = parts[0]
    x1 = parts[1] if len(parts) > 1 else None
    cin0, d, h, w = x0.shape
    up = 2 if upsample else 1
    pad = 1 if ksize == 3 else 0
    od = (d * up + 2 * pad - ksize) // stride + 1
    oh = (h * up + 2 * pad - ksize) // stride + 1
    ow = (w * up + 2 * pad - ksize) // stride + 1
    desc = ConvDesc()
    if out_size is not None:
        od, oh, ow = min(od, int(out_size[0])), min(oh, int(out_size[1])), min(ow, int(out_size[2]))
        desc.out_d, desc.out_h, desc.out_w = od, oh, ow
    out = alloc((cout, od, oh, ow), torch.float32)
    desc.d_in0 = addr(x0); desc.c0 = cin0
    desc.d_in1 = addr(x1)
    desc.c1 = x1.shape[0] if x1 is not None else 0
    desc.in_d, desc.in_h, desc.in_w = d, h, w
    desc.upsample = 1 if upsample else 0
    desc.stride = stride
    desc.ksize = ksize
    desc.d_pro_a = addr(pro[0]) if pro is not None else None
    desc.d_pro_b = addr(pro[1]) if pro is not None else None
    desc.d_gamma = addr(affine[0]) if affine is not None else None
    desc.d_beta = addr(affine[1]) if affine is not None else None
    desc.act = act
    desc.d_w = addr(packed_w)
    desc.d_w16 = addr(w16)
    desc.w16_subpixel = 1 if subpixel else 0
    desc.d_in_amax0 = addr(in_amax[0]) if in_amax else None
    desc.d_in_amax1 = addr(in_amax[1]) if in_amax and len(in_amax) > 1 else None
    desc.in_bound = float(in_bound)
    desc.d_bias = addr(bias)
    desc.c_out = cout
    desc.d_residual = addr(residual)
    desc.d_out = addr(out)
    if skip is not None:
        sp = skip["parts"]
        desc.d_skip_in0 = addr(sp[0]); desc.skip_c0 = sp[0].shape[0]
        desc.d_skip_in1 = addr(sp[1]) if len(sp) > 1 else None
        desc.skip_c1 = sp[1].shape[0] if len(sp) > 1 else 0
        desc.d_skip_w16 = addr(skip["w16"])
        desc.d_skip_bias = addr(skip["bias"])
        desc.d_skip_amax0 = addr(skip["amax"][0])
        desc.d_skip_amax1 = addr(skip["amax"][1]) if len(sp) > 1 else None
    stats = workspace = None
    if w16 is not None and split_k:
        wsb = lib.pixie_conv_workspace_bytes(C.byref(desc))
        if wsb > 0:
            workspace = alloc((wsb,), torch.uint8)
            desc.d_workspace = addr(workspace)
    if out_amax is not None and w16 is not None:
        nfl = lib.pixie_conv_stats_floats(C.byref(desc))
        if nfl > 0 and (workspace is None or split_stats):
            stats = alloc((nfl,), torch.float32)
            desc.d_out_stats = addr(stats)
            desc.d_out_amax = addr(out_amax)
    return desc, out, stats, workspace


class PendingStats:

    def __init__(self, stats: torch.Tensor, desc: ConvDesc, cout: int):
        self.stats, self.desc, self.cout = stats, desc, cout


class HipOps:

    def __init__(self, device: torch.device):
        if device.type != "cuda":
            raise _lib.PixieHipError("pixie_amd U-Net operators run on a HIP device only (no CPU fallback)")
        self.device = device
        self.lib = _lib.load()
        self.split_k = os.environ.get("PIXIE_CONV_SPLIT_K", "1") != "0"
        self.record_variant = False
        self.last_variant = (0, 1)

    @property
    def stream(self):
        return _lib.current_stream_ptr()

    def pack_conv(self, weight: torch.Tensor) -> torch.Tensor:
        cout, cin = weight.shape[0], weight.shape[1]
        k = weight.shape[2]
        coutp = self.lib.pixie_conv_cout_padded(cout)
        w = weight.detach().to(self.device, torch.float32).contiguous()
        taps = 1
        for s in weight.shape[2:]:
            taps *= int(s)
        packed = torch.empty((taps, cin, coutp), device=self.device, dtype=torch.float32)
        check(self.lib.pixie_conv_pack_weights(_ptr(w), _ptr(packed), cout, cin, k, self.stream), "pixie_conv_pack_weights")
        return packed

    def pack_conv16(self, weight: torch.Tensor) -> torch.Tensor:
        cout, cin, k = weight.shape[0], weight.shape[1], weight.shape[2]
        nbytes = self.lib.pixie_conv_packed16_bytes(cout, cin, k)
        if nbytes <= 0:
            raise _lib.PixieHipError(f"f16x3 packing needs c_in % 8 == 0 (got {cin})")
        w = weight.detach().to(self.device, torch.float32).contiguous()
        packed = torch.empty(nbytes, device=self.device, dtype=torch.uint8)
        check(self.lib.pixie_conv_pack_weights_f16x2(_ptr(w), _ptr(packed), cout, cin, k, self.stream), "pixie_conv_pack_weights_f16x2")
        return packed

    def pack_conv_subpixel(self, weight: torch.Tensor) -> torch.Tensor:
        cout, cin = weight.shape[0], weight.shape[1]
        nbytes = self.lib.pixie_conv_subpixel_bytes(cout, cin) if tuple(weight.shape[2:]) == (3, 3, 3) else 0
        if nbytes <= 0:
            raise _lib.PixieHipError(f"sub-pixel packing needs a 3x3x3 weight with c_in % 16 == 0 (got {tuple(weight.shape)})")
        w = weight.detach().to(self.device, torch.float32).contiguous()
        packed = torch.empty(nbytes, device=self.device, dtype=torch.uint8)
        check(self.lib.pixie_conv_pack_weights_subpixel(_ptr(w), _ptr(packed), cout, cin, self.stream), "pixie_conv_pack_weights_subpixel")
        return packed

    @staticmethod
    def f16x3_ok(parts: Sequence[torch.Tensor], stride: int) -> bool:
        cin = sum(int(p.shape[0]) for p in parts)
        return stride in (1, 2) and cin % 16 == 0 and int(parts[0].shape[0]) % 8 == 0

    def conv(self, parts: Sequence[torch.Tensor], packed_w: Optional[torch.Tensor], bias: Optional[torch.Tensor], cout: int, ksize: int,
             stride: int = 1, upsample: bool = False, pro: Optional[Tuple[torch.Tensor, torch.Tensor]] = None,
             affine: Optional[Tuple[torch.Tensor, torch.Tensor]] = None, act: int = ACT_NONE,
             residual: Optional[torch.Tensor] = None, w16: Optional[torch.Tensor] = None,
             in_amax: Optional[Sequence[torch.Tensor]] = None, in_bound: float = 0.0,
             out_amax: Optional[torch.Tensor] = None, out_size: Optional[Tuple[int, int, int]] = None,
             skip: Optional[dict] = None, subpixel: bool = False, defer_stats: bool = False, split_stats: bool = True):
        desc, out, stats, _ = fill_conv_desc(
            self.lib, lambda shape, dtype: torch.empty(shape, device=self.device, dtype=dtype), parts, packed_w, bias, cout, ksize,
            stride=stride, upsample=upsample, pro=pro, affine=affine, act=act, residual=residual, w16=w16, in_amax=in_amax,
            in_bound=in_bound, out_amax=out_amax, out_size=out_size, skip=skip, subpixel=subpixel, split_k=self.split_k,
            split_stats=defer_stats and split_stats)
        sums = None
        if self.record_variant:
            sl = C.c_int(1)
            self.last_variant = (int(_lib.load(diag=True).pixie_conv_kernel_variant(C.byref(desc), C.byref(sl))), int(sl.value))
        check(self.lib.pixie_conv3d_forward(C.byref(desc), self.stream), "pixie_conv3d_forward")
        if desc.d_out_stats:
            if defer_stats:
                sums = PendingStats(stats, desc, cout)
            else:
                sums = self.stats_finalize(PendingStats(stats, desc, cout))
        if out_amax is not None:
            return out, sums
        return out

    def skip_foldable(self, x: torch.Tensor, cout: int, ksize: int, skip_parts: Sequence[torch.Tensor]) -> bool:
        desc = ConvDesc()
        desc.c0 = x.shape[0]
        desc.in_d, desc.in_h, desc.in_w = (int(v) for v in x.shape[1:])
        desc.stride, desc.ksize, desc.c_out = 1, ksize, cout
        desc.d_w16 = 1
        desc.d_workspace = 1 if self.split_k else None
        desc.skip_c0 = skip_parts[0].shape[0]
        desc.skip_c1 = skip_parts[1].shape[0] if len(skip_parts) > 1 else 0
        return bool(self.lib.pixie_conv_skip_foldable(C.byref(desc)))

    def channel_sums(self, x: torch.Tensor) -> torch.Tensor:
        c = x.shape[0]
        spatial = x.numel() // c
        sums = torch.empty((c, 2), device=self.device, dtype=torch.float64)
        check(self.lib.pixie_channel_sums(_ptr(x), c, spatial, _ptr(sums), self.stream), "pixie_channel_sums")
        return sums

    def channel_stats(self, x: torch.Tensor, amax_slot: torch.Tensor) -> torch.Tensor:
        c = x.shape[0]
        spatial = x.numel() // c
        sums = torch.empty((c, 2), device=self.device, dtype=torch.float64)
        check(self.lib.pixie_channel_stats(_ptr(x), c, spatial, _ptr(sums), _ptr(amax_slot), self.stream), "pixie_channel_stats")
        return sums

    def norm_finalize(self, sums: torch.Tensor, spatial: int, mode: int, groups: int = 1, eps: float = 1e-5,
                      weight: Optional[torch.Tensor] = None, bias: Optional[torch.Tensor] = None):
        c = sums.shape[0]
        a = torch.empty(c, device=self.device, dtype=torch.float32)
        b = torch.empty(c, device=self.device, dtype=torch.float32)
        check(self.lib.pixie_norm_finalize(_ptr(sums), c, spatial, mode, groups, eps, _ptr(weight), _ptr(bias), _ptr(a), _ptr(b),
                                           self.stream), "pixie_norm_finalize")
        return a, b

    def stats_finalize(self, pending: PendingStats) -> torch.Tensor:
        sums = torch.empty((pending.cout, 2), device=self.device, dtype=torch.float64)
        check(self.lib.pixie_stats_finalize(_ptr(pending.stats), C.byref(pending.desc), _ptr(sums), self.stream), "pixie_stats_finalize")
        return sums

    def stats_norm_finalize(self, parts: Sequence, spatial: int, mode: int, groups: int = 1, eps: float = 1e-5,
                            weight: Optional[torch.Tensor] = None, bias: Optional[torch.Tensor] = None):
        pend = [isinstance(p, PendingStats) for p in parts]
        sums = [torch.empty((p.cout, 2), device=self.device, dtype=torch.float64) if is_p else p for p, is_p in zip(parts, pend)]
        c0 = sums[0].shape[0]
        c1 = sums[1].shape[0] if len(parts) > 1 else 0
        if pend[0]:
            desc0 = parts[0].desc
        else:
            desc0 = ConvDesc()
            desc0.c_out = c0
        two = len(parts) > 1
        a = torch.empty(c0 + c1, device=self.device, dtype=torch.float32)
        b = torch.empty(c0 + c1, device=self.device, dtype=torch.float32)
        check(self.lib.pixie_stats_norm_finalize(
            _ptr(parts[0].stats) if pend[0] else None, C.byref(desc0), _ptr(sums[0]),
            _ptr(parts[1].stats) if two and pend[1] else None, C.byref(parts[1].desc) if two and pend[1] else None,
            _ptr(sums[1]) if two else None, c1, spatial, mode, groups, eps, _ptr(weight), _ptr(bias), _ptr(a), _ptr(b), self.stream),
            "pixie_stats_norm_finalize")
        return a, b, sums

    def attention(self, qkv: torch.Tensor, channels: int, tokens: int) -> torch.Tensor:
        out = torch.empty((channels, tokens), device=self.device, dtype=torch.float32)
        check(self.lib.pixie_attention_forward(_ptr(qkv), _ptr(out), channels, tokens, self.stream), "pixie_attention_forward")
        return out

    def projector_conv0(self, grid_dhwc_f16: torch.Tensor, nets: Sequence[Tuple[torch.Tensor, Optional[torch.Tensor]]], cout: int):
        d, h, w, c = (int(v) for v in grid_dhwc_f16.shape)
        g = grid_dhwc_f16.contiguous()
        outs = [torch.empty((cout, d, h, w), device=self.device, dtype=torch.float32) for _ in nets]
        n = len(nets)
        w_arr = (C.c_void_p * n)(*[t[0].data_ptr() for t in nets])
        b_arr = (C.c_void_p * n)(*[(t[1].data_ptr() if t[1] is not None else None) for t in nets])
        o_arr = (C.c_void_p * n)(*[o.data_ptr() for o in outs])
        check(self.lib.pixie_projector_conv0(_ptr(g), d * h * w, c, n, w_arr, b_arr, o_arr, cout, self.stream), "pixie_projector_conv0")
        return outs

    def combine(self, logits: torch.Tensor, cont: torch.Tensor):
        ncls = logits.shape[0]
        spatial = logits.numel() // ncls
        combined = torch.empty((3 + ncls,) + tuple(logits.shape[1:]), device=self.device, dtype=torch.float32)
        amax = torch.empty(tuple(logits.shape[1:]), device=self.device, dtype=torch.int32)
        check(self.lib.pixie_combine_predictions(_ptr(logits), ncls, _ptr(cont), spatial, _ptr(combined), _ptr(amax), self.stream),
              "pixie_combine_predictions")
        return combined, amax


class UNetRunner:

    def __init__(self, cfg: UNetConfig, params: Dict[str, torch.Tensor], ops, precision: Optional[str] = None):
        self.cfg = cfg
        self.plan: UNetPlan = build_plan(cfg)
        self.p = params
        self.ops = ops
        self.precision = precision or DEFAULT_PRECISION
        if self.precision not in ("f16x3", "f32"):
            raise ValueError(f"unknown conv precision {self.precision!r}")
        self._packed: Dict[str, Tuple[int, int, torch.Tensor]] = {}
        self._packed16: Dict[str, Tuple[int, int, torch.Tensor]] = {}
        self._bounds: Dict[str, Tuple[int, int, float, float]] = {}
        self.fuse_stats = os.environ.get("PIXIE_FUSE_STATS", "1") != "0"
        self.fold_skip = os.environ.get("PIXIE_FOLD_SKIP", "1") != "0"
        self.subpixel = os.environ.get("PIXIE_CONV_SUBPIXEL", "1") != "0"
        self.split_stats = os.environ.get("PIXIE_SPLIT_STATS", "1") != "0"

    @property
    def _f16x3(self) -> bool:
        return self.precision == "f16x3" and hasattr(self.ops, "pack_conv16")

    def _w(self, key: str) -> torch.Tensor:
        t = self.p[key + ".weight"]
        ent = self._packed.get(key)
        if ent is None or ent[0] != t.data_ptr() or ent[1] != t._version:
            self._packed[key] = (t.data_ptr(), t._version, self.ops.pack_conv(t))
        return self._packed[key][2]

    def _w16(self, key: str, subpixel: bool = False) -> torch.Tensor:
        t = self.p[key + ".weight"]
        ck = key + "#subpixel" if subpixel else key
        ent = self._packed16.get(ck)
        if ent is None or ent[0] != t.data_ptr() or ent[1] != t._version:
            self._packed16[ck] = (t.data_ptr(), t._version, self.ops.pack_conv_subpixel(t) if subpixel else self.ops.pack_conv16(t))
        return self._packed16[ck][2]

    def _b(self, key: str) -> torch.Tensor:
        return self.p[key + ".bias"]

    def _absmax(self, key: str) -> Tuple[float, float]:
        w, bb = self.p[key + ".weight"], self.p[key + ".bias"]
        ent = self._bounds.get(key)
        if ent is None or ent[0] != w._version or ent[1] != bb._version:
            self._bounds[key] = (w._version, bb._version, float(w.abs().max()), float(bb.abs().max()))
            ent = self._bounds[key]
        return ent[2], ent[3]

    def _norm_bound(self, key: str, count: int) -> float:
        wmax, bmax = self._absmax(key)
        return math.sqrt(float(count)) * wmax + bmax + 1e-30

    _SLOT_POOL = 1024

    @classmethod
    def _new_slot(cls, cache: dict, device) -> torch.Tensor:
        pool = cache.get("_slots")
        if pool is None or cache["_next"] >= pool.numel():
            pool = cache["_slots"] = torch.zeros(cls._SLOT_POOL, dtype=torch.int32, device=device)
            cache["_next"] = 0
        i = cache["_next"]
        cache["_next"] = i + 1
        return pool[i:i + 1]

    @staticmethod
    def _remember(cache: dict, t: torch.Tensor, sums, slot) -> None:
        k = id(t)
        cache[k] = (sums, slot)
        weakref.finalize(t, cache.pop, k, None)

    def _stats(self, cache: dict, t: torch.Tensor):
        k = id(t)
        if k not in cache:
            if hasattr(self.ops, "channel_stats"):
                slot = self._new_slot(cache, t.device)
                self._remember(cache, t, self.ops.channel_stats(t, slot), slot)
            else:
                self._remember(cache, t, self.ops.channel_sums(t), None)
        if isinstance(cache[k][0], PendingStats):
            cache[k] = (self.ops.stats_finalize(cache[k][0]), cache[k][1])
        return cache[k]

    def _norm(self, cache: dict, parts: List[torch.Tensor], spatial: int, mode: int, groups: int = 1, weight=None, bias=None):
        ops = self.ops
        for t in parts:
            if id(t) not in cache:
                self._stats(cache, t)
        ents = [cache[id(t)][0] for t in parts]
        if any(isinstance(e, PendingStats) for e in ents):
            a, b, sums = ops.stats_norm_finalize(ents, spatial, mode, groups=groups, weight=weight, bias=bias)
            for t, sm in zip(parts, sums):
                cache[id(t)] = (sm, cache[id(t)][1])
            return a, b
        sums = torch.cat(ents, dim=0) if len(ents) > 1 else ents[0]
        if mode == 0:
            return ops.norm_finalize(sums, spatial, 0)
        return ops.norm_finalize(sums, spatial, mode, groups=groups, weight=weight, bias=bias)

    def _sums(self, cache: dict, t: torch.Tensor) -> torch.Tensor:
        return self._stats(cache, t)[0]

    def _amax(self, cache: dict, t: torch.Tensor) -> torch.Tensor:
        k = id(t)
        return cache[k][1] if k in cache else self._stats(cache, t)[1]

    def _conv(self, cache: dict, parts: List[torch.Tensor], wkey: str, cout: int, ksize: int, *, stride: int = 1,
              upsample: bool = False, pro=None, affine_key: Optional[str] = None, act: int = ACT_NONE,
              residual: Optional[torch.Tensor] = None, bound: float = 0.0, out_size=None, skip=None) -> torch.Tensor:
        ops = self.ops
        affine = (self.p[affine_key + ".weight"], self.p[affine_key + ".bias"]) if affine_key else None
        if not (self._f16x3 and ops.f16x3_ok(parts, stride)):
            return ops.conv(parts, self._w(wkey), self._b(wkey), cout, ksize, stride=stride, upsample=upsample, pro=pro,
                            affine=affine, act=act, residual=residual, **({"out_size": out_size} if out_size is not None else {}))
        if pro is None and affine is None:
            kw = dict(in_amax=[self._amax(cache, t) for t in parts])
        else:
            kw = dict(in_bound=bound)
        if out_size is not None:
            kw["out_size"] = out_size
        if skip is not None:
            kw["skip"] = skip
        sub = self.subpixel and upsample and ksize == 3 and stride == 1 and hasattr(ops, "pack_conv_subpixel")
        if sub:
            kw["subpixel"] = True
        if self.fuse_stats:
            slot = self._new_slot(cache, parts[0].device)
            if hasattr(ops, "stats_norm_finalize"):
                kw["defer_stats"] = True
                kw["split_stats"] = self.split_stats
            out, sums = ops.conv(parts, None, self._b(wkey), cout, ksize, stride=stride, upsample=upsample, pro=pro, affine=affine,
                                 act=act, residual=residual, w16=self._w16(wkey, sub), out_amax=slot, **kw)
            if sums is not None:
                self._remember(cache, out, sums, slot)
            return out
        return ops.conv(parts, None, self._b(wkey), cout, ksize, stride=stride, upsample=upsample, pro=pro, affine=affine,
                        act=act, residual=residual, w16=self._w16(wkey, sub), **kw)

    def _res(self, b: Block, parts: List[torch.Tensor], cache: dict) -> torch.Tensor:
        ops, p = self.ops, b.prefix
        spatial = parts[0][0].numel()
        pro = self._norm(cache, parts, spatial, 0)
        h = self._conv(cache, parts, p + ".in_layers.2", b.cout, 3, pro=pro, affine_key=p + ".in_layers.0", act=ACT_LEAKY,
                       bound=self._norm_bound(p + ".in_layers.0", spatial))
        pro2 = self._norm(cache, [h], spatial, 0)
        fold = None
        if b.cin != b.cout:
            if (self.fold_skip and self._f16x3 and ops.f16x3_ok([h], 1) and ops.f16x3_ok(parts, 1)
                    and ops.skip_foldable(h, b.cout, 3, parts)):
                skip = None
                fold = dict(parts=parts, w16=self._w16(p + ".skip_connection"), bias=self._b(p + ".skip_connection"),
                            amax=[self._amax(cache, t) for t in parts])
            else:
                skip = self._conv(cache, parts, p + ".skip_connection", b.cout, 1)
        else:
            skip = parts[0]
        return self._conv(cache, [h], p + ".out_layers.3", b.cout, 3, pro=pro2, affine_key=p + ".out_layers.0", act=ACT_LEAKY,
                          residual=skip, bound=self._norm_bound(p + ".out_layers.0", spatial), skip=fold)

    def _attn(self, b: Block, x: torch.Tensor, cache: dict) -> torch.Tensor:
        ops, p = self.ops, b.prefix
        c = x.shape[0]
        spatial = x[0].numel()
        pro = self._norm(cache, [x], spatial, 1, groups=32, weight=self.p[p + ".norm.weight"], bias=self.p[p + ".norm.bias"])
        qkv = self._conv(cache, [x], p + ".qkv", 3 * c, 1, pro=pro, bound=self._norm_bound(p + ".norm", spatial * (c // 32)))
        att = ops.attention(qkv.reshape(3 * c, spatial), c, spatial).reshape(x.shape)
        return self._conv(cache, [att], p + ".proj_out", c, 1, residual=x)

    def _block(self, b: Block, parts: List[torch.Tensor], cache: dict, up_size=None) -> torch.Tensor:
        if b.kind == "res":
            return self._res(b, parts, cache)
        assert len(parts) == 1
        x = parts[0]
        if b.kind == "attn":
            return self._attn(b, x, cache)
        if b.kind == "down":
            return self._conv(cache, [x], b.prefix + ".op", b.cout, 3, stride=2)
        if b.kind == "up":
            return self._conv(cache, [x], b.prefix + ".conv", b.cout, 3, upsample=True, out_size=up_size)
        raise ValueError(b.kind)

    def _stem(self, feat: Optional[torch.Tensor], cache: dict, proj0: Optional[torch.Tensor] = None) -> torch.Tensor:
        cfg, ops = self.cfg, self.ops
        spatial = (proj0 if proj0 is not None else feat)[0].numel()
        x = feat
        pro_in, act_in, bound_in = None, ACT_NONE, 0.0
        if cfg.has_projector:
            q = "projector.net."
            if cfg.projector_hidden is None:
                g = max(cfg.cond_dim // 2, 1)
                x = self._conv(cache, [x], q + "0", cfg.cond_dim, 1)
                pro_in = self._norm(cache, [x], spatial, 1, groups=g, weight=self.p[q + "1.weight"], bias=self.p[q + "1.bias"])
                act_in = ACT_SILU
                bound_in = self._norm_bound(q + "1", spatial * (cfg.cond_dim // g))
            else:
                hid = cfg.projector_hidden
                x = proj0 if proj0 is not None else self._conv(cache, [x], q + "0", hid, 1)
                pro = self._norm(cache, [x], spatial, 1, groups=32, weight=self.p[q + "1.weight"], bias=self.p[q + "1.bias"])
                x = self._conv(cache, [x], q + "3", hid, 3, pro=pro, act=ACT_SILU, bound=self._norm_bound(q + "1", spatial * (hid // 32)))
                pro = self._norm(cache, [x], spatial, 1, groups=32, weight=self.p[q + "4.weight"], bias=self.p[q + "4.bias"])
                x = self._conv(cache, [x], q + "6", cfg.cond_dim, 1, pro=pro, act=ACT_SILU, bound=self._norm_bound(q + "4", spatial * (hid // 32)))
                pro_in = self._norm(cache, [x], spatial, 1, groups=32, weight=self.p[q + "7.weight"], bias=self.p[q + "7.bias"])
                bound_in = self._norm_bound(q + "7", spatial * max(cfg.cond_dim // 32, 1))
        first = self.plan.input_blocks[0][0]
        return self._conv(cache, [x], first.prefix, first.cout, 3, pro=pro_in, act=act_in, bound=bound_in)

    def _head(self, h: torch.Tensor, cache: dict) -> torch.Tensor:
        pro = self._norm(cache, [h], h[0].numel(), 0)
        return self._conv(cache, [h], "unet.out.2", self.cfg.out_channels, 3, pro=pro, affine_key="unet.out.0", act=ACT_LEAKY,
                          bound=self._norm_bound("unet.out.0", h[0].numel()))

    def forward(self, feat: Optional[torch.Tensor], taps: Optional[dict] = None, proj0: Optional[torch.Tensor] = None) -> torch.Tensor:
        cache: dict = {}
        only = set(taps) if taps else None

        def tap(key, t):
            if taps is not None and (only is None or key in only):
                taps[key] = t

        plan = self.plan
        hs: List[torch.Tensor] = []
        h = self._stem(feat, cache, proj0)
        hs.append(h)
        tap("unet.input_blocks.0", h)
        for seq in plan.input_blocks[1:]:
            for b in seq:
                h = self._block(b, [h], cache)
            hs.append(h)
            tap(seq[0].prefix.rsplit(".", 1)[0], h)
        for b in plan.middle:
            h = self._block(b, [h], cache)
            tap(b.prefix, h)
        for seq in plan.output_blocks:
            skip = hs.pop()
            assert tuple(skip.shape[1:]) == tuple(h.shape[1:]), (skip.shape, h.shape)
            parts = [h, skip]
            for b in seq:
                h = self._block(b, parts, cache, up_size=tuple(hs[-1].shape[1:]) if (b.kind == "up" and hs) else None)
                parts = [h]
            tap(seq[0].prefix.rsplit(".", 1)[0], h)
        return self._head(h, cache)


class UNetHandle:

    def __init__(self, cfg: UNetConfig, precision: str, device: torch.device):
        if device.type != "cuda":
            raise _lib.PixieHipError("pixie_amd U-Net runs on a HIP device only (no CPU fallback)")
        if precision not in ("f16x3", "f32"):
            raise ValueError(f"unknown conv precision {precision!r}")
        self.lib = _lib.load()
        self.cfg, self.precision, self.device = cfg, precision, device
        c = _lib.UNetConfigC()
        c.feature_channels, c.cond_dim, c.model_channels, c.num_res_blocks = cfg.feature_channels, cfg.cond_dim, cfg.model_channels, cfg.num_res_blocks
        c.n_channel_mult = len(cfg.channel_mult)
        for i, m in enumerate(cfg.channel_mult):
            c.channel_mult[i] = int(m)
        c.n_attention_resolutions = len(cfg.attention_resolutions)
        for i, m in enumerate(cfg.attention_resolutions):
            c.attention_resolutions[i] = int(m)
        c.grid_size, c.out_channels, c.precision = cfg.grid_size, cfg.out_channels, 0 if precision == "f16x3" else 1
        self._h = C.c_void_p()
        check(self.lib.pixie_unet_create(C.byref(self._h), C.byref(c)), "pixie_unet_create")
        weakref.finalize(self, self.lib.pixie_unet_destroy, self._h)
        self._seen: Dict[str, Tuple[int, int]] = {}
        self._keep: Dict[str, torch.Tensor] = {}

    def keys(self) -> List[str]:
        out = []
        for i in range(self.lib.pixie_unet_param_count(self._h)):
            key = C.c_char_p()
            check(self.lib.pixie_unet_param_info(self._h, i, C.byref(key), None, None, None), "pixie_unet_param_info")
            out.append(key.value.decode())
        return out

    def load(self, params: Dict[str, torch.Tensor]) -> None:
        for key, t in params.items():
            tag = (t.data_ptr(), t._version)
            if self._seen.get(key) == tag:
                continue
            v = t.detach()
            if v.device != self.device or v.dtype != torch.float32 or not v.is_contiguous():
                v = v.to(self.device, torch.float32).contiguous()
            self._keep[key] = v
            check(self.lib.pixie_unet_set_param(self._h, key.encode(), _ptr(v), v.numel()), "pixie_unet_set_param")
            self._seen[key] = tag

    def workspace_bytes(self, d: int, h: int, w: int) -> int:
        n = int(self.lib.pixie_unet_workspace_bytes(self._h, d, h, w))
        if n < 0:
            raise _lib.PixieHipError(self.lib.pixie_last_error().decode())
        return n

    def forward(self, feat: Optional[torch.Tensor], proj0: Optional[torch.Tensor] = None, workspace: Optional[torch.Tensor] = None) -> torch.Tensor:
        src = proj0 if proj0 is not None else feat
        d, h, w = (int(v) for v in src.shape[1:])
        out = torch.empty((self.cfg.out_channels, d, h, w), device=self.device, dtype=torch.float32)
        nbytes = self.workspace_bytes(d, h, w)
        if workspace is None:
            workspace = torch.empty(nbytes, device=self.device, dtype=torch.uint8)
        elif workspace.dtype != torch.uint8 or workspace.device != self.device or workspace.numel() < nbytes or not workspace.is_contiguous():
            raise ValueError(f"workspace must be a contiguous uint8 tensor of >= {nbytes} bytes on {self.device}")
        check(self.lib.pixie_unet_forward(self._h, _ptr(feat), _ptr(proj0), d, h, w, _ptr(out), _ptr(workspace), nbytes,
                                          _lib.current_stream_ptr()), "pixie_unet_forward")
        return out


class _Node(nn.Module):
    """Empty container used to reproduce the reference's state_dict key hierarchy."""


class _PixieUNet(nn.Module):
    def __init__(self, cfg: UNetConfig):
        super().__init__()
        self.cfg = cfg
        shapes = param_shapes(cfg)
        gen = torch.Generator().manual_seed(0)
        for key, shape in shapes.items():
            parts = key.split(".")
            node = self
            for name in parts[:-1]:
                if name not in node._modules:
                    node.add_module(name, _Node())
                node = node._modules[name]
            node.register_parameter(parts[-1], nn.Parameter(self._init(key, shape, shapes, gen), requires_grad=False))
        self._runner: Optional[UNetRunner] = None
        self._handle: Optional[UNetHandle] = None
        self.executor = os.environ.get("PIXIE_UNET_EXECUTOR", "c")
        self.conv_precision = DEFAULT_PRECISION
        self.use_graph = os.environ.get("PIXIE_UNET_GRAPH", "1") == "1"
        self._graphs: dict = {}
        self._plist = None

    @staticmethod
    def _init(key, shape, shapes, gen) -> torch.Tensor:
        if is_norm_key(key):
            return torch.ones(shape) if key.endswith(".weight") else torch.zeros(shape)
        if key.endswith(_ZERO_INIT_SUFFIXES):
            return torch.zeros(shape)
        wshape = shapes[key[: key.rfind(".")] + ".weight"]
        bound = 1.0 / math.sqrt(float(torch.tensor(wshape[1:]).prod()))
        return (torch.rand(shape, generator=gen) * 2.0 - 1.0) * bound

    def _params(self) -> Dict[str, torch.Tensor]:
        return {k: v for k, v in self.named_parameters()}

    def load_numpy_state(self, sd) -> None:
        self.load_state_dict({k: torch.from_numpy(v) for k, v in sd.items()}, strict=True)

    @torch.no_grad()
    def forward(self, feat_grid: torch.Tensor, taps: Optional[dict] = None) -> torch.Tensor:
        if feat_grid.dim() != 5 or feat_grid.shape[1] != self.cfg.feature_channels:
            raise ValueError(f"expected (N,{self.cfg.feature_channels},D,H,W), got {tuple(feat_grid.shape)}")
        dev = next(self.parameters()).device
        if dev.type != "cuda" or feat_grid.device != dev:
            raise _lib.PixieHipError("model and input must live on the same HIP device (no CPU fallback)")
        with torch.cuda.device(dev):
            self._prepare(dev)
            x = feat_grid.detach().to(torch.float32).contiguous()
            if self.use_graph and taps is None:
                return torch.stack([self._forward_graphed(x[n]) for n in range(x.shape[0])], dim=0)
            outs = [self._forward_one(x[n], taps=taps if n == 0 else None) for n in range(x.shape[0])]
            return torch.stack(outs, dim=0)

    def _prepare(self, dev) -> None:
        params = self._params()
        if self._runner is None or self._runner.ops.device != dev or self._runner.precision != self.conv_precision:
            self._runner = UNetRunner(self.cfg, params, HipOps(dev), precision=self.conv_precision)
        else:
            self._runner.p = params
        if self.executor == "c":
            if self._handle is None or self._handle.device != dev or self._handle.precision != self.conv_precision:
                self._handle = UNetHandle(self.cfg, self.conv_precision, dev)
            self._handle.load(params)
        elif self.executor != "python":
            raise ValueError(f"unknown executor {self.executor!r} (PIXIE_UNET_EXECUTOR is 'c' or 'python')")

    def _forward_one(self, x: Optional[torch.Tensor], taps: Optional[dict] = None, proj0: Optional[torch.Tensor] = None) -> torch.Tensor:
        if self.executor == "c" and taps is None:
            return self._handle.forward(x, proj0)
        return self._runner.forward(x, taps, proj0)

    def _apply(self, fn, *args, **kwargs):
        self._plist = None
        return super()._apply(fn, *args, **kwargs)

    def _param_list(self) -> List[torch.Tensor]:
        refs = self.__dict__.get("_plist")
        if refs is None:
            refs = self._plist = [(m._parameters, name) for m in self.modules() for name, p in m._parameters.items() if p is not None]
        return [d[name] for d, name in refs]

    def load_state_dict(self, state_dict, strict: bool = True, assign: bool = False):
        self._plist = None
        return super().load_state_dict(state_dict, strict=strict, assign=assign)

    def _forward_graphed(self, x: Optional[torch.Tensor], proj0: Optional[torch.Tensor] = None) -> torch.Tensor:
        src = proj0 if proj0 is not None else x
        base = (tuple(src.shape), tuple(src.stride()), src.dtype, proj0 is not None, self.executor, self.conv_precision, src.device.index,
                tuple((id(p), p.data_ptr(), p._version) for p in self._param_list()))
        run = (lambda t: self._forward_one(None, proj0=t)) if proj0 is not None else (lambda t: self._forward_one(t))
        if self._graphs.get("base") != base:
            self._graphs = {"base": base, "first_ptr": None}
        ent = self._graphs.get(src.data_ptr()) or self._graphs.get("copy")
        if ent is None:
            out = run(src)
            if self._graphs["first_ptr"] is None:
                self._graphs["first_ptr"] = src.data_ptr()
                return out
            in_place = (proj0 is None and self._graphs["first_ptr"] == src.data_ptr() and "copy" not in self._graphs
                        and os.environ.get("PIXIE_UNET_GRAPH_INPLACE", "1") == "1")
            try:
                static_in = src if in_place else src.clone()
                side = torch.cuda.Stream(src.device)
                side.wait_stream(torch.cuda.current_stream())
                with torch.cuda.stream(side):
                    run(static_in)
                torch.cuda.current_stream().wait_stream(side)
                graph = torch.cuda.CUDAGraph()
                with torch.cuda.graph(graph, capture_error_mode="thread_local"):
                    static_out = run(static_in)
            except RuntimeError as exc:
                warnings.warn(f"pixie_amd: HIP-graph capture of the U-Net forward failed ({exc}); continuing with eager launches",
                              RuntimeWarning)
                self.use_graph = False
                return out
            if in_place:
                ent = self._graphs[src.data_ptr()] = (graph, None, static_out)
            else:
                ent = self._graphs["copy"] = (graph, static_in, static_out)
        graph, static_in, static_out = ent
        if static_in is not None:
            static_in.copy_(src)
        graph.replay()
        return static_out.clone()


class SegmentationUNet(_PixieUNet):

    def __init__(self, feature_channels: int, cond_dim: int, model_channels: int, num_res_blocks: int,
                 channel_mult: Tuple[int, ...], attention_resolutions: Tuple[int, ...], grid_size: int, num_classes: int):
        super().__init__(UNetConfig(feature_channels, cond_dim, model_channels, num_res_blocks, tuple(channel_mult),
                                    tuple(attention_resolutions), grid_size, num_classes))


class RegressionUNet(_PixieUNet):

    def __init__(self, feature_channels: int, cond_dim: int, model_channels: int, num_res_blocks: int,
                 channel_mult: Tuple[int, ...], attention_resolutions: Tuple[int, ...], grid_size: int, out_channels: int = 3):
        super().__init__(UNetConfig(feature_channels, cond_dim, model_channels, num_res_blocks, tuple(channel_mult),
                                    tuple(attention_resolutions), grid_size, out_channels))


@torch.no_grad()
def predict_material_field_from_voxel_grid(seg_network: "SegmentationUNet", cont_network: "RegressionUNet", grid_dhwc_f16: torch.Tensor,
                                           dual_stream: Optional[bool] = None):
    dev = next(seg_network.parameters()).device
    g = grid_dhwc_f16
    if g.dim() != 4 or g.dtype != torch.float16 or g.device != dev or dev.type != "cuda":
        raise ValueError("expected a (D, H, W, C) float16 tensor on the networks' HIP device")
    nets = (seg_network, cont_network)
    for net in nets:
        if net.cfg.projector_hidden is None or net.cfg.feature_channels != g.shape[3] or net.conv_precision != "f16x3":
            raise ValueError("the fused grid path needs the hidden-128 projector, matching feature_channels and conv_precision 'f16x3'")
        net._prepare(dev)
    ops = seg_network._runner.ops
    q = "projector.net.0"
    packed = [(net._runner._w16(q), net._runner._b(q)) for net in nets]
    x_seg, x_cont = ops.projector_conv0(g, packed, seg_network.cfg.projector_hidden)
    if dual_stream is None:
        dual_stream = _dual_stream_default(seg_network, cont_network, int(g.shape[0]) * int(g.shape[1]) * int(g.shape[2]))

    def fwd(net, p0):
        return net._forward_graphed(None, p0) if net.use_graph else net._forward_one(None, proj0=p0)

    if dual_stream:
        cur = torch.cuda.current_stream()
        s1, s2 = _side_streams(dev)
        s1.wait_stream(cur); s2.wait_stream(cur)
        with torch.cuda.stream(s1):
            seg_logits = fwd(seg_network, x_seg)[None]
        with torch.cuda.stream(s2):
            cont_pred = fwd(cont_network, x_cont)[None]
        x_seg.record_stream(s1); x_cont.record_stream(s2)
        cur.wait_stream(s1); cur.wait_stream(s2)
        seg_logits.record_stream(cur); cont_pred.record_stream(cur)
    else:
        seg_logits = fwd(seg_network, x_seg)[None]
        cont_pred = fwd(cont_network, x_cont)[None]
    combined, seg_pred = ops.combine(seg_logits[0].contiguous(), cont_pred[0].contiguous())
    return combined[None], seg_pred[None], seg_logits, cont_pred


_SIDE_STREAMS: Dict[str, Tuple[torch.cuda.Stream, torch.cuda.Stream]] = {}


def _dual_stream_default(seg_network, cont_network, voxels: int) -> bool:
    env = os.environ.get("PIXIE_DUAL_STREAM")
    if env is not None:
        return env == "1"
    return not (seg_network.use_graph and cont_network.use_graph and voxels >= 128 ** 3)


def _side_streams(device):
    key = str(device)
    if key not in _SIDE_STREAMS:
        _SIDE_STREAMS[key] = (torch.cuda.Stream(device), torch.cuda.Stream(device))
    return _SIDE_STREAMS[key]


@torch.no_grad()
def predict_material_field(seg_network: SegmentationUNet, cont_network: RegressionUNet, feat_grid: torch.Tensor,
                           dual_stream: Optional[bool] = None):
    if feat_grid.is_cuda and feat_grid.device.index != torch.cuda.current_device():
        with torch.cuda.device(feat_grid.device):
            return predict_material_field(seg_network, cont_network, feat_grid, dual_stream)
    if dual_stream is None:
        dual_stream = _dual_stream_default(seg_network, cont_network, int(feat_grid[0, 0].numel()))
    if dual_stream and feat_grid.is_cuda:
        cur = torch.cuda.current_stream()
        s1, s2 = _side_streams(feat_grid.device)
        s1.wait_stream(cur); s2.wait_stream(cur)
        with torch.cuda.stream(s1):
            seg_logits = seg_network(feat_grid)
        with torch.cuda.stream(s2):
            cont_pred = cont_network(feat_grid)
        feat_grid.record_stream(s1); feat_grid.record_stream(s2)
        cur.wait_stream(s1); cur.wait_stream(s2)
        seg_logits.record_stream(cur); cont_pred.record_stream(cur)
    else:
        seg_logits = seg_network(feat_grid)
        cont_pred = cont_network(feat_grid)
    ops = seg_network._runner.ops
    combined, seg_pred = [], []
    for n in range(feat_grid.shape[0]):
        cmb, am = ops.combine(seg_logits[n].contiguous(), cont_pred[n].contiguous())
        combined.append(cmb)
        seg_pred.append(am)
    return torch.stack(combined), torch.stack(seg_pred), seg_logits, cont_pred
```

Measured before the change: 24.81 million voxels/s.

## Share projector conv0 across both U-Nets with fused f32 split and tile statistics

Adds a fused kernel that reads the f32 CDHW feature grid once, splits it to fp16 hi/lo with an amax-based scale, and computes the first projector conv for both segmentation and regression networks in one pass. The same kernel writes per-tile sum/sumsq statistics and an output |x| max, so the following norm layer can finalize from tile partials without re-reading the output. A new U-Net entry point consumes these precomputed outputs and stats, and the default predict path uses this shared route. This removes a duplicate read of the 64-channel grid and a separate stats pass, at the cost of extra amax and zeroing launches and more complex graph-capture keying.

```diff
diff --git a/include/pixie_hip.h b/include/pixie_hip.h
--- a/include/pixie_hip.h
+++ b/include/pixie_hip.h
@@ -133,6 +133,9 @@
 int pixie_stats_norm_finalize(const float* d_stats0, const pixie_conv_desc* desc0, double* d_sums0, const float* d_stats1,
                               const pixie_conv_desc* desc1, double* d_sums1, int c1, int64_t spatial, int mode, int groups,
                               double eps, const float* d_weight, const float* d_bias, float* d_a, float* d_b, void* stream);
+int pixie_stats_norm_finalize_tiles(const float* d_stats, int64_t n_tiles, int c_out_padded, int channels, double* d_sums, int64_t spatial,
+                                    int mode, int groups, double eps, const float* d_weight, const float* d_bias, float* d_a, float* d_b,
+                                    void* stream);
 int pixie_conv_skip_foldable(const pixie_conv_desc* desc);
 
 int pixie_channel_sums(const float* d_x, int channels, int64_t spatial, double* d_sums, void* stream);
@@ -150,6 +153,11 @@
 
 int pixie_projector_conv0(const void* d_feat_dhwc_f16, int64_t voxels, int channels, int n_networks, const void* const* d_w16,
                           const float* const* d_bias, float* const* d_out, int c_out, void* stream);
+
+int64_t pixie_projector_conv0_f32_stats_floats(int64_t voxels, int c_out);
+int pixie_projector_conv0_f32(const float* d_feat_cdhw, int64_t voxels, int channels, int n_networks, const void* const* d_w16,
+                              const float* const* d_bias, float* const* d_out, int c_out, const uint32_t* d_in_amax,
+                              float* const* d_out_stats, uint32_t* const* d_out_amax, void* stream);
 
 int pixie_pack_fields(const float* d_cont, const int32_t* d_seg_pred, int64_t n_scenes, int64_t spatial, void* d_wire, int64_t wire_bytes,
                       void* stream);
@@ -178,6 +186,8 @@
 int64_t pixie_unet_workspace_bytes(pixie_unet* h, int d, int hh, int w);
 int pixie_unet_forward(pixie_unet* h, const float* d_feat, const float* d_proj0, int d, int hh, int w, float* d_out,
                        void* d_workspace, int64_t workspace_bytes, void* stream);
+int pixie_unet_forward_proj0(pixie_unet* h, const float* d_proj0, const float* d_proj0_stats, const uint32_t* d_proj0_amax, int d, int hh,
+                             int w, float* d_out, void* d_workspace, int64_t workspace_bytes, void* stream);
 int pixie_unet_set_option(pixie_unet* h, const char* key, int value);
 
 typedef struct pixie_field_desc {
diff --git a/pixie_amd/_lib.py b/pixie_amd/_lib.py
--- a/pixie_amd/_lib.py
+++ b/pixie_amd/_lib.py
@@ -137,6 +137,9 @@
     "pixie_attention_forward": (_I, [_VP, _VP, _I, _I, _VP]),
     "pixie_channel_affine": (_I, [_VP, _VP, _VP, _VP, _I, _I64, _VP]),
     "pixie_projector_conv0": (_I, [_VP, _I64, _I, _I, C.POINTER(_VP), C.POINTER(_VP), C.POINTER(_VP), _I, _VP]),
+    "pixie_projector_conv0_f32_stats_floats": (_I64, [_I64, _I]),
+    "pixie_projector_conv0_f32": (_I, [_VP, _I64, _I, _I, C.POINTER(_VP), C.POINTER(_VP), C.POINTER(_VP), _I, _VP, C.POINTER(_VP), C.POINTER(_VP), _VP]),
+    "pixie_stats_norm_finalize_tiles": (_I, [_VP, _I64, _I, _I, _VP, _I64, _I, _I, _D, _VP, _VP, _VP, _VP, _VP]),
     "pixie_conv_skip_foldable": (_I, [C.POINTER(ConvDesc)]),
     "pixie_unet_create": (_I, [C.POINTER(_VP), C.POINTER(UNetConfigC)]),
     "pixie_unet_destroy": (_I, [_VP]),
@@ -146,6 +149,7 @@
     "pixie_unet_workspace_bytes": (_I64, [_VP, _I, _I, _I]),
     "pixie_unet_set_option": (_I, [_VP, _S, _I]),
     "pixie_unet_forward": (_I, [_VP, _VP, _VP, _I, _I, _I, _VP, _VP, _I64, _VP]),
+    "pixie_unet_forward_proj0": (_I, [_VP, _VP, _VP, _VP, _I, _I, _I, _VP, _VP, _I64, _VP]),
     "pixie_combine_class_ids": (_I, [_VP, _I, _VP, _I64, _VP, _VP]),
     "pixie_combine_predictions": (_I, [_VP, _I, _VP, _I64, _VP, _VP, _VP]),
     "pixie_voxel_grid_to_ncdhw": (_I, [_VP, _I, _I, _I, _I, _VP, _VP]),
diff --git a/pixie_amd/csrc/conv3d_f16x3.hip b/pixie_amd/csrc/conv3d_f16x3.hip
--- a/pixie_amd/csrc/conv3d_f16x3.hip
+++ b/pixie_amd/csrc/conv3d_f16x3.hip
@@ -1112,6 +1112,20 @@
     return 0;
 }
 
+extern "C" int pixie_stats_norm_finalize_tiles(const float* d_stats, int64_t n_tiles, int c_out_padded, int channels, double* d_sums, int64_t spatial,
+                                               int mode, int groups, double eps, const float* d_weight, const float* d_bias, float* d_a, float* d_b,
+                                               void* stream) {
+    PX_REQUIRE(d_stats && d_sums && d_a && d_b && spatial > 0 && n_tiles > 0 && n_tiles <= 0x7fffffff, "pixie_stats_norm_finalize_tiles: bad arguments");
+    PX_REQUIRE(channels > 0 && channels <= c_out_padded, "pixie_stats_norm_finalize_tiles: %d channels in rows of %d", channels, c_out_padded);
+    PX_REQUIRE(mode == 0 || (mode == 1 && groups > 0 && channels % groups == 0), "pixie_stats_norm_finalize_tiles: bad mode/groups");
+    const StatParts none{nullptr, 0, 0, 0, 0};
+    const StatParts p0{d_stats, (int)n_tiles, (long)n_tiles, 1, 0};
+    hipLaunchKernelGGL(stats_norm_finalize_kernel, dim3((unsigned)(mode == 0 ? channels : groups)), dim3(256), 0, as_stream(stream), p0, d_sums, channels,
+                       none, static_cast<double*>(nullptr), channels, (double)spatial, mode, groups, eps, d_weight, d_bias, d_a, d_b);
+    PX_CHECK_HIP(hipGetLastError());
+    return 0;
+}
+
 extern "C" int64_t pixie_conv_packed16_bytes(int c_out, int c_in, int ksize) {
     if (c_out <= 0 || c_in <= 0 || c_in % 8 != 0 || (ksize != 1 && ksize != 3)) return 0;
     const int64_t taps = (int64_t)ksize * ksize * ksize;
diff --git a/pixie_amd/csrc/projector_fused.hip b/pixie_amd/csrc/projector_fused.hip
--- a/pixie_amd/csrc/projector_fused.hip
+++ b/pixie_amd/csrc/projector_fused.hip
@@ -1,4 +1,6 @@
 #include <hip/hip_runtime.h>
+
+#include <algorithm>
 
 #include "../../include/pixie_hip.h"
 #include "common.h"
@@ -97,6 +99,174 @@
                 if (v < A.voxels) out[(size_t)co * A.voxels + v] = acc[mb][nb][r] * inv + bv;
             }
         }
+}
+
+
+constexpr int kFNV = 128;
+constexpr int kFLDO = kFNV + 4;
+
+__device__ __forceinline__ int p_scale_exponent(float bound) {
+    const unsigned bits = __float_as_uint(bound);
+    const int eb = (int)((bits >> 23) & 0xffu) - 127;
+    if (!(bound > 0.0f) || eb > 100) return 0;
+    int e = 14 - eb;
+    return e > 100 ? 100 : (e < -100 ? -100 : e);
+}
+__device__ __forceinline__ float p_pow2i(int e) { return __uint_as_float((unsigned)(e + 127) << 23); }
+
+struct Proj32Args {
+    const float* x;
+    long voxels;
+    int C, KG;
+    int coutp, cout;
+    int vec;
+    const uint4* w16[kPMaxNets];
+    const float* bias[kPMaxNets];
+    float* out[kPMaxNets];
+    float* stats[kPMaxNets];
+    unsigned* amax[kPMaxNets];
+    const unsigned* in_amax;
+};
+
+__global__ __launch_bounds__(256, 2) void projector_conv0_f32_kernel(Proj32Args A) {
+    extern __shared__ uint4 xs[];
+    const int tid = threadIdx.x, lane = tid & 63, wave = tid >> 6;
+    const int kh = lane >> 5, l31 = lane & 31;
+    const int row0 = wave * 64;
+    const int net = row0 / A.coutp, co0 = row0 % A.coutp;
+    const long v0 = (long)blockIdx.x * kFNV;
+
+    const int ex = p_scale_exponent(__uint_as_float(*A.in_amax));
+    const float sx = p_pow2i(ex);
+
+    f32x16 acc[2][4];
+#pragma unroll
+    for (int mb = 0; mb < 2; ++mb)
+#pragma unroll
+        for (int nb = 0; nb < 4; ++nb)
+#pragma unroll
+            for (int r = 0; r < 16; ++r) acc[mb][nb][r] = 0.0f;
+
+    uint4* xhi = xs;
+    uint4* xlo = xs + 8 * kFNV;
+    const uint4* wHi = A.w16[net] + kPW16HeaderU4 + co0 + l31;
+    const size_t lo_off = (size_t)A.KG * A.coutp;
+    const int svox = tid & (kFNV - 1), sg = tid >> 7;
+    const bool sok = v0 + svox < A.voxels;
+    const float* xv = A.x + (sok ? v0 + svox : 0);
+
+    for (int c_base = 0; c_base < A.C; c_base += kPKC) {
+        __syncthreads();
+        float val[4][8];
+#pragma unroll
+        for (int q = 0; q < 4; ++q) {
+            const int c = c_base + 8 * (sg + 2 * q);
+#pragma unroll
+            for (int j = 0; j < 8; ++j) val[q][j] = c < A.C ? xv[(size_t)(c + j) * A.voxels] : 0.0f;
+        }
+#pragma unroll
+        for (int q = 0; q < 4; ++q) {
+            f16x8 vh, vl;
+#pragma unroll
+            for (int j = 0; j < 8; ++j) {
+                const float t = val[q][j] + 0.0f;
+                const float sc = sok ? t * sx : 0.0f;
+                const _Float16 h = (_Float16)sc;
+                vh[j] = h;
+                vl[j] = (_Float16)(sc - (float)h);
+            }
+            xhi[(sg + 2 * q) * kFNV + svox] = __builtin_bit_cast(uint4, vh);
+            xlo[(sg + 2 * q) * kFNV + svox] = __builtin_bit_cast(uint4, vl);
+        }
+        __syncthreads();
+#pragma unroll 2
+        for (int ks = 0; ks < kPKC / 16; ++ks) {
+            if (c_base + 16 * ks >= A.C) break;
+            const size_t kg = (size_t)((c_base >> 3) + 2 * ks + kh);
+            f16x8 ah[2], al[2], bh[4], bl[4];
+#pragma unroll
+            for (int mb = 0; mb < 2; ++mb) {
+                ah[mb] = __builtin_bit_cast(f16x8, wHi[kg * A.coutp + mb * 32]);
+                al[mb] = __builtin_bit_cast(f16x8, wHi[lo_off + kg * A.coutp + mb * 32]);
+            }
+#pragma unroll
+            for (int nb = 0; nb < 4; ++nb) {
+                bh[nb] = __builtin_bit_cast(f16x8, xhi[(2 * ks + kh) * kFNV + nb * 32 + l31]);
+                bl[nb] = __builtin_bit_cast(f16x8, xlo[(2 * ks + kh) * kFNV + nb * 32 + l31]);
+            }
+#pragma unroll
+            for (int mb = 0; mb < 2; ++mb)
+#pragma unroll
+                for (int nb = 0; nb < 4; ++nb) acc[mb][nb] = __builtin_amdgcn_mfma_f32_32x32x16_f16(al[mb], bh[nb], acc[mb][nb], 0, 0, 0);
+#pragma unroll
+            for (int mb = 0; mb < 2; ++mb)
+#pragma unroll
+                for (int nb = 0; nb < 4; ++nb) acc[mb][nb] = __builtin_amdgcn_mfma_f32_32x32x16_f16(ah[mb], bl[nb], acc[mb][nb], 0, 0, 0);
+#pragma unroll
+            for (int mb = 0; mb < 2; ++mb)
+#pragma unroll
+                for (int nb = 0; nb < 4; ++nb) acc[mb][nb] = __builtin_amdgcn_mfma_f32_32x32x16_f16(ah[mb], bh[nb], acc[mb][nb], 0, 0, 0);
+        }
+    }
+
+    __syncthreads();
+    float* ldsO = reinterpret_cast<float*>(xs) + wave * (32 * kFLDO);
+    const float inv = __uint_as_float(A.w16[net][0].x) * p_pow2i(-ex);
+    float* out = A.out[net];
+    const float* bias = A.bias[net];
+    float* stats = A.stats[net];
+    const int colq = 4 * l31;
+    const long vq = v0 + colq;
+    const bool ok0 = vq < A.voxels, ok1 = vq + 1 < A.voxels, ok2 = vq + 2 < A.voxels, ok3 = vq + 3 < A.voxels;
+    float wmax = 0.0f;
+#pragma unroll
+    for (int mb = 0; mb < 2; ++mb) {
+#pragma unroll
+        for (int r = 0; r < 16; ++r)
+#pragma unroll
+            for (int nb = 0; nb < 4; ++nb) ldsO[((r & 3) + 8 * (r >> 2) + 4 * kh) * kFLDO + nb * 32 + l31] = acc[mb][nb][r];
+#pragma unroll 4
+        for (int it = 0; it < 16; ++it) {
+            const int rowl = 2 * it + kh;
+            const int co = co0 + mb * 32 + rowl;
+            const bool rok = co < A.cout;
+            const float4 a4 = *reinterpret_cast<const float4*>(ldsO + rowl * kFLDO + colq);
+            const float bv = (bias && rok) ? bias[co] : 0.0f;
+            float4 v4;
+            v4.x = a4.x * inv + bv; v4.y = a4.y * inv + bv; v4.z = a4.z * inv + bv; v4.w = a4.w * inv + bv;
+            if (rok) {
+                float* o = out + (size_t)co * A.voxels + vq;
+                if (A.vec && ok3) {
+                    *reinterpret_cast<float4*>(o) = v4;
+                } else {
+                    if (ok0) o[0] = v4.x;
+                    if (ok1) o[1] = v4.y;
+                    if (ok2) o[2] = v4.z;
+                    if (ok3) o[3] = v4.w;
+                }
+            }
+            if (stats) {
+                const float x = ok0 ? v4.x : 0.0f, y = ok1 ? v4.y : 0.0f, z = ok2 ? v4.z : 0.0f, w = ok3 ? v4.w : 0.0f;
+                float s1 = (x + y) + (z + w);
+                float s2 = (x * x + y * y) + (z * z + w * w);
+                wmax = fmaxf(fmaxf(wmax, fmaxf(fabsf(x), fabsf(y))), fmaxf(fabsf(z), fabsf(w)));
+#pragma unroll
+                for (int off = 16; off > 0; off >>= 1) { s1 += __shfl_xor(s1, off, 64); s2 += __shfl_xor(s2, off, 64); }
+                if (l31 == 0) *reinterpret_cast<float2*>(stats + ((size_t)co * gridDim.x + blockIdx.x) * 2) = make_float2(s1, s2);
+            }
+        }
+    }
+    if (stats && A.amax[net]) {
+#pragma unroll
+        for (int off = 32; off > 0; off >>= 1) wmax = fmaxf(wmax, __shfl_xor(wmax, off, 64));
+        const unsigned m = __float_as_uint(wmax);
+        if (lane == 0 && m > __hip_atomic_load(A.amax[net], __ATOMIC_RELAXED, __HIP_MEMORY_SCOPE_AGENT)) atomicMax(A.amax[net], m);
+    }
+}
+
+__global__ void projector_zero_slots_kernel(unsigned* s0, unsigned* s1) {
+    if (threadIdx.x == 0 && s0) *s0 = 0u;
+    if (threadIdx.x == 1 && s1) *s1 = 0u;
 }
 
 }
@@ -130,3 +300,49 @@
     PX_CHECK_HIP(hipGetLastError());
     return 0;
 }
+
+extern "C" int64_t pixie_projector_conv0_f32_stats_floats(int64_t voxels, int c_out) {
+    if (voxels <= 0 || c_out <= 0) return 0;
+    return (voxels + kFNV - 1) / kFNV * (int64_t)pixie_conv_cout_padded(c_out) * 2;
+}
+
+extern "C" int pixie_projector_conv0_f32(const float* d_feat_cdhw, int64_t voxels, int channels, int n_networks, const void* const* d_w16,
+                                         const float* const* d_bias, float* const* d_out, int c_out, const uint32_t* d_in_amax,
+                                         float* const* d_out_stats, uint32_t* const* d_out_amax, void* stream) {
+    PX_REQUIRE(d_feat_cdhw && d_w16 && d_out && d_in_amax && voxels > 0, "pixie_projector_conv0_f32: null argument");
+    PX_REQUIRE(n_networks >= 1 && n_networks <= kPMaxNets, "pixie_projector_conv0_f32: 1 or 2 networks");
+    PX_REQUIRE(channels > 0 && channels % 16 == 0, "pixie_projector_conv0_f32: the channel count must be a multiple of 16 (got %d)", channels);
+    const int coutp = pixie_conv_cout_padded(c_out);
+    PX_REQUIRE(c_out > 0 && n_networks * coutp == 256, "pixie_projector_conv0_f32: %d x %d output rows are not the tiling this kernel has (256)", n_networks, coutp);
+    PX_REQUIRE((d_out_stats == nullptr) == (d_out_amax == nullptr), "pixie_projector_conv0_f32: d_out_stats and d_out_amax come together");
+    Proj32Args a{};
+    a.x = d_feat_cdhw;
+    a.voxels = voxels; a.C = channels; a.KG = channels / 8;
+    a.coutp = coutp; a.cout = c_out;
+    a.in_amax = d_in_amax;
+    a.vec = voxels % 4 == 0;
+    for (int n = 0; n < n_networks; ++n) {
+        PX_REQUIRE(d_w16[n] && d_out[n], "pixie_projector_conv0_f32: null weights / output for network %d", n);
+        a.w16[n] = static_cast<const uint4*>(d_w16[n]);
+        a.bias[n] = d_bias ? d_bias[n] : nullptr;
+        a.out[n] = d_out[n];
+        if (reinterpret_cast<size_t>(d_out[n]) & 15) a.vec = 0;
+        if (d_out_stats) {
+            PX_REQUIRE(d_out_stats[n] && d_out_amax[n], "pixie_projector_conv0_f32: null statistics buffer / |x|max slot for network %d", n);
+            PX_REQUIRE((reinterpret_cast<size_t>(d_out_stats[n]) & 7) == 0, "pixie_projector_conv0_f32: d_out_stats must be 8-byte aligned");
+            a.stats[n] = d_out_stats[n];
+            a.amax[n] = d_out_amax[n];
+        }
+    }
+    hipStream_t st = as_stream(stream);
+    if (d_out_stats) {
+        hipLaunchKernelGGL(projector_zero_slots_kernel, dim3(1), dim3(64), 0, st, a.amax[0], a.amax[1]);
+        PX_CHECK_HIP(hipGetLastError());
+    }
+    const size_t lds = std::max((size_t)16 * kFNV * sizeof(uint4), (size_t)4 * 32 * kFLDO * sizeof(float));
+    PX_CHECK_HIP(allow_max_dynamic_lds(reinterpret_cast<const void*>(projector_conv0_f32_kernel)));
+    const long tiles = (voxels + kFNV - 1) / kFNV;
+    hipLaunchKernelGGL(projector_conv0_f32_kernel, dim3((unsigned)tiles), dim3(256), lds, st, a);
+    PX_CHECK_HIP(hipGetLastError());
+    return 0;
+}
diff --git a/pixie_amd/csrc/unet_exec.hip b/pixie_amd/csrc/unet_exec.hip
--- a/pixie_amd/csrc/unet_exec.hip
+++ b/pixie_amd/csrc/unet_exec.hip
@@ -218,6 +218,8 @@
     double* sums = nullptr;
     int64_t partials_off = -1;
     pixie_conv_desc pdesc;
+    const float* ext_partials = nullptr;
+    int64_t ext_tiles = 0;
     uint32_t* slot = nullptr;
     int64_t spatial() const { return (int64_t)d * h * w; }
     ~Tens();
@@ -242,10 +244,10 @@
     std::unordered_map<std::string, Bound> bounds;
     uint32_t* d_bound_slots = nullptr;
     std::vector<uint32_t> h_bound_slots;
-    std::map<std::tuple<int, int, int, bool>, Sized> sized;
+    std::map<std::tuple<int, int, int, int>, Sized> sized;
     bool fuse_stats = true, split_k = true, fold_skip = true, subpixel = true;
     bool split_stats = true;
-    struct Replay { const float* feat; const float* proj0; float* out; void* ws; int d; uint64_t epoch; hipGraph_t graph; hipGraphExec_t exec; };
+    struct Replay { const float* feat; const float* proj0; const float* p0stats; float* out; void* ws; int d; uint64_t epoch; hipGraph_t graph; hipGraphExec_t exec; };
     bool use_graph = false;
     uint64_t epoch = 0;
     std::vector<Replay> replays;
@@ -343,7 +345,7 @@
     }
 
     void stats(const TP& t) {
-        if (t->has_sums || t->partials_off >= 0) return;
+        if (t->has_sums || t->partials_off >= 0 || t->ext_partials) return;
         t->has_sums = true;
         if (!dry && zsum_next + 2 * t->c > zsum_cap) fail("pixie_unet_forward: out of statistics space (internal sizing error)");
         t->sums = dry ? nullptr : zsums + zsum_next;
@@ -363,7 +365,12 @@
         r.a = r.mem->as<float>();
         r.b = r.a + cpad;
         const bool p0 = t0->partials_off >= 0, p1 = t1 && t1->partials_off >= 0;
-        if (p0 || p1) {
+        if (t0->ext_partials) {
+            if (t1) fail("pixie_unet_forward: a tensor with caller-owned partial statistics cannot be part of a concatenation");
+            if (!dry) ok(pixie_stats_norm_finalize_tiles(t0->ext_partials, t0->ext_tiles, pixie_conv_cout_padded(c0), c0, t0->sums, spatial, mode, groups,
+                                                         1e-5, w, b, r.a, r.b, stream), "pixie_stats_norm_finalize_tiles");
+            parts[0]->ext_partials = nullptr; parts[0]->has_sums = true;
+        } else if (p0 || p1) {
             pixie_conv_desc d0 = t0->pdesc;
             if (!p0) { std::memset(&d0, 0, sizeof d0); d0.c_out = c0; }
             if (!dry) ok(pixie_stats_norm_finalize(p0 ? arena.ptr<float>(t0->partials_off) : nullptr, &d0, t0->sums,
@@ -523,7 +530,7 @@
         fail("pixie_unet: unexpected block kind");
     }
 
-    TP forward(const float* d_feat, const float* d_proj0, int D, int H, int W, float* d_out) {
+    TP forward(const float* d_feat, const float* d_proj0, const float* d_p0stats, const uint32_t* d_p0amax, int D, int H, int W, float* d_out) {
         const Cfg& c = net->cfg;
         const int64_t spatial = (int64_t)D * H * W;
         TP x;
@@ -539,7 +546,15 @@
                 act_in = ACT_SILU;
                 bound_in = norm_bound(q + "1", spatial * (c.cond_dim / g));
             } else {
-                if (d_proj0) x = external(d_proj0, hid, D, H, W);
+                if (d_proj0) {
+                    x = external(d_proj0, hid, D, H, W);
+                    if (d_p0stats) {
+                        x->ext_partials = d_p0stats; x->ext_tiles = (spatial + 127) / 128;
+                        x->slot = const_cast<uint32_t*>(d_p0amax);
+                        x->sums_off = arena.alloc((int64_t)hid * 2 * sizeof(double));
+                        x->sums = arena.ptr<double>(x->sums_off);
+                    }
+                }
                 else x = conv({external(d_feat, c.feature_channels, D, H, W)}, q + "0", hid, 1, ConvOpt{});
                 AB pro = norm_finalize({x}, spatial, 1, 32, P(q + "1.weight"), P(q + "1.bias"));
                 ConvOpt o; o.pro = &pro; o.act = ACT_SILU; o.bound = norm_bound(q + "1", spatial * (hid / 32));
@@ -638,8 +653,9 @@
 int64_t slot_region_bytes(int n_slots) { return ((int64_t)n_slots * 4 + kSlotAlign - 1) / kSlotAlign * kSlotAlign; }
 int64_t zsum_region_bytes(int64_t n_doubles) { return (n_doubles * 8 + kSlotAlign - 1) / kSlotAlign * kSlotAlign; }
 
-Sized size_pass(pixie_unet* net, int D, int H, int W, bool from_proj0) {
-    auto key = std::make_tuple(D, H, W, from_proj0);
+Sized size_pass(pixie_unet* net, int D, int H, int W, int entry) {
+    const bool from_proj0 = entry != 0;
+    auto key = std::make_tuple(D, H, W, entry);
     auto it = net->sized.find(key);
     if (it != net->sized.end()) return it->second;
     Exec ex;
@@ -647,7 +663,8 @@
     ex.arena.reset(reinterpret_cast<char*>(0x10000000), (int64_t)1 << 50);
     {
         const float* fake = reinterpret_cast<const float*>(0x100);
-        TP out = ex.forward(from_proj0 ? nullptr : fake, from_proj0 ? fake : nullptr, D, H, W, reinterpret_cast<float*>(0x100));
+        TP out = ex.forward(from_proj0 ? nullptr : fake, from_proj0 ? fake : nullptr, entry == 2 ? fake : nullptr,
+                            entry == 2 ? reinterpret_cast<const uint32_t*>(0x100) : nullptr, D, H, W, reinterpret_cast<float*>(0x100));
     }
     Sized r{ex.arena.peak + slot_region_bytes(ex.slot_next) + zsum_region_bytes(ex.zsum_next), ex.slot_next, ex.zsum_next};
     net->sized[key] = r;
@@ -727,22 +744,22 @@
     if (!h || d <= 0 || hh <= 0 || w <= 0) { set_error("pixie_unet_workspace_bytes: bad argument"); return -1; }
     int64_t bytes = -1;
     const int rc = guarded([&] {
-        bytes = size_pass(h, d, hh, w, false).bytes;
-        if (h->cfg.projector_hidden() > 0) bytes = std::max(bytes, size_pass(h, d, hh, w, true).bytes);
+        bytes = size_pass(h, d, hh, w, 0).bytes;
+        if (h->cfg.projector_hidden() > 0) bytes = std::max({bytes, size_pass(h, d, hh, w, 1).bytes, size_pass(h, d, hh, w, 2).bytes});
         return 0;
     });
     return rc == 0 ? bytes : -1;
 }
 
-extern "C" int pixie_unet_forward(pixie_unet* h, const float* d_feat, const float* d_proj0, int d, int hh, int w, float* d_out,
-                                  void* d_workspace, int64_t workspace_bytes, void* stream) {
+static int unet_forward(pixie_unet* h, const float* d_feat, const float* d_proj0, const float* d_p0stats, const uint32_t* d_p0amax, int d, int hh,
+                        int w, float* d_out, void* d_workspace, int64_t workspace_bytes, void* stream) {
     PX_REQUIRE(h && d_out && d_workspace && (d_feat || d_proj0), "pixie_unet_forward: null argument");
     PX_REQUIRE(d == h->cfg.grid_size && hh == d && w == d,
                "pixie_unet_forward: the network was built for a %d^3 grid (its LayerNorm parameters have that shape), got %d x %d x %d", h->cfg.grid_size, d, hh, w);
     PX_REQUIRE(!d_proj0 || h->cfg.projector_hidden() > 0, "pixie_unet_forward: d_proj0 needs the hidden-128 projector (feature_channels > cond_dim)");
     PX_REQUIRE(d_feat || (d_proj0 && h->cfg.has_projector()), "pixie_unet_forward: d_feat is null");
     return guarded([&] {
-        const auto sized = size_pass(h, d, hh, w, d_proj0 != nullptr);
+        const auto sized = size_pass(h, d, hh, w, d_proj0 ? (d_p0stats ? 2 : 1) : 0);
         if (workspace_bytes < sized.bytes)
             fail("pixie_unet_forward: workspace of %lld bytes, this grid needs %lld (pixie_unet_workspace_bytes)", (long long)workspace_bytes, (long long)sized.bytes);
         auto launch_all = [&] {
@@ -757,12 +774,12 @@
                                static_cast<uint4*>(d_workspace), head_bytes / 16);
             if (hipGetLastError() != hipSuccess) fail("pixie_unet_forward: clearing the workspace head failed");
             ex.arena.reset(static_cast<char*>(d_workspace) + head_bytes, workspace_bytes - head_bytes);
-            TP out = ex.forward(d_feat, d_proj0, d, hh, w, d_out);
+            TP out = ex.forward(d_feat, d_proj0, d_p0stats, d_p0amax, d, hh, w, d_out);
         };
         if (h->use_graph) {
             for (size_t i = 0; i < h->replays.size(); ++i) {
                 const pixie_unet::Replay& r = h->replays[i];
-                if (r.feat != d_feat || r.proj0 != d_proj0 || r.out != d_out || r.ws != d_workspace || r.d != d) continue;
+                if (r.feat != d_feat || r.proj0 != d_proj0 || r.p0stats != d_p0stats || r.out != d_out || r.ws != d_workspace || r.d != d) continue;
                 if (r.epoch != h->epoch) { h->drop_replay(i); break; }
                 if (hipGraphLaunch(r.exec, as_stream(stream)) != hipSuccess) fail("pixie_unet_forward: hipGraphLaunch failed: %s", hipGetErrorString(hipGetLastError()));
                 if (i + 1 != h->replays.size()) std::rotate(h->replays.begin() + (long)i, h->replays.begin() + (long)i + 1, h->replays.end());
@@ -784,10 +801,21 @@
             hipGraphExec_t exec = nullptr;
             if (hipGraphInstantiate(&exec, graph, nullptr, nullptr, 0) != hipSuccess) { (void)hipGraphDestroy(graph); fail("pixie_unet_forward: hipGraphInstantiate failed"); }
             if (h->replays.size() >= pixie_unet::kMaxReplays) h->drop_replay(0);
-            h->replays.push_back(pixie_unet::Replay{d_feat, d_proj0, d_out, d_workspace, d, h->epoch, graph, exec});
+            h->replays.push_back(pixie_unet::Replay{d_feat, d_proj0, d_p0stats, d_out, d_workspace, d, h->epoch, graph, exec});
         }
         return 0;
     });
+}
+
+extern "C" int pixie_unet_forward(pixie_unet* h, const float* d_feat, const float* d_proj0, int d, int hh, int w, float* d_out,
+                                  void* d_workspace, int64_t workspace_bytes, void* stream) {
+    return unet_forward(h, d_feat, d_proj0, nullptr, nullptr, d, hh, w, d_out, d_workspace, workspace_bytes, stream);
+}
+
+extern "C" int pixie_unet_forward_proj0(pixie_unet* h, const float* d_proj0, const float* d_proj0_stats, const uint32_t* d_proj0_amax, int d, int hh,
+                                        int w, float* d_out, void* d_workspace, int64_t workspace_bytes, void* stream) {
+    PX_REQUIRE(d_proj0 && d_proj0_stats && d_proj0_amax, "pixie_unet_forward_proj0: null argument");
+    return unet_forward(h, nullptr, d_proj0, d_proj0_stats, d_proj0_amax, d, hh, w, d_out, d_workspace, workspace_bytes, stream);
 }
 
 extern "C" int pixie_unet_set_option(pixie_unet* h, const char* key, int value) {
diff --git a/pixie_amd/unet.py b/pixie_amd/unet.py
--- a/pixie_amd/unet.py
+++ b/pixie_amd/unet.py
@@ -97,6 +97,12 @@
         self.stats, self.desc, self.cout = stats, desc, cout
 
 
+class PendingTileStats:
+
+    def __init__(self, stats: torch.Tensor, slot: torch.Tensor, cout: int):
+        self.stats, self.slot, self.cout = stats, slot, cout
+
+
 class HipOps:
 
     def __init__(self, device: torch.device):
@@ -235,6 +241,18 @@
             "pixie_stats_norm_finalize")
         return a, b, sums
 
+    def tile_stats_norm_finalize(self, pending: PendingTileStats, spatial: int, mode: int, groups: int = 1, eps: float = 1e-5,
+                                 weight: Optional[torch.Tensor] = None, bias: Optional[torch.Tensor] = None):
+        c = pending.cout
+        coutp = self.lib.pixie_conv_cout_padded(c)
+        sums = torch.empty((c, 2), device=self.device, dtype=torch.float64)
+        a = torch.empty(c, device=self.device, dtype=torch.float32)
+        b = torch.empty(c, device=self.device, dtype=torch.float32)
+        check(self.lib.pixie_stats_norm_finalize_tiles(_ptr(pending.stats), pending.stats.numel() // (2 * coutp), coutp, c, _ptr(sums), spatial, mode,
+                                                       groups, eps, _ptr(weight), _ptr(bias), _ptr(a), _ptr(b), self.stream),
+              "pixie_stats_norm_finalize_tiles")
+        return a, b, sums
+
     def attention(self, qkv: torch.Tensor, channels: int, tokens: int) -> torch.Tensor:
         out = torch.empty((channels, tokens), device=self.device, dtype=torch.float32)
         check(self.lib.pixie_attention_forward(_ptr(qkv), _ptr(out), channels, tokens, self.stream), "pixie_attention_forward")
@@ -250,6 +268,25 @@
         o_arr = (C.c_void_p * n)(*[o.data_ptr() for o in outs])
         check(self.lib.pixie_projector_conv0(_ptr(g), d * h * w, c, n, w_arr, b_arr, o_arr, cout, self.stream), "pixie_projector_conv0")
         return outs
+
+    def tensor_amax(self, x: torch.Tensor, slot: torch.Tensor) -> None:
+        check(self.lib.pixie_tensor_amax(_ptr(x), x.numel(), _ptr(slot), self.stream), "pixie_tensor_amax")
+
+    def projector_conv0_f32(self, feat: torch.Tensor, nets: Sequence[Tuple[torch.Tensor, Optional[torch.Tensor]]], cout: int,
+                            in_amax: torch.Tensor, outs: Optional[Sequence[torch.Tensor]] = None,
+                            stats: Optional[Sequence[torch.Tensor]] = None, out_amax: Optional[Sequence[torch.Tensor]] = None):
+        c, d, h, w = (int(v) for v in feat.shape)
+        n = len(nets)
+        if outs is None:
+            outs = [torch.empty((cout, d, h, w), device=self.device, dtype=torch.float32) for _ in nets]
+        arr = lambda ts: (C.c_void_p * n)(*[(t.data_ptr() if t is not None else None) for t in ts])
+        check(self.lib.pixie_projector_conv0_f32(_ptr(feat), d * h * w, c, n, arr([t[0] for t in nets]), arr([t[1] for t in nets]), arr(outs), cout,
+                                                 _ptr(in_amax), arr(stats) if stats is not None else None,
+                                                 arr(out_amax) if out_amax is not None else None, self.stream), "pixie_projector_conv0_f32")
+        return list(outs)
+
+    def conv0_stats_floats(self, voxels: int, cout: int) -> int:
+        return int(self.lib.pixie_projector_conv0_f32_stats_floats(voxels, cout))
 
     def combine(self, logits: torch.Tensor, cont: torch.Tensor):
         ncls = logits.shape[0]
@@ -349,6 +386,11 @@
             if id(t) not in cache:
                 self._stats(cache, t)
         ents = [cache[id(t)][0] for t in parts]
+        if isinstance(ents[0], PendingTileStats):
+            assert len(parts) == 1
+            a, b, sm = ops.tile_stats_norm_finalize(ents[0], spatial, mode, groups=groups, weight=weight, bias=bias)
+            cache[id(parts[0])] = (sm, cache[id(parts[0])][1])
+            return a, b
         if any(isinstance(e, PendingStats) for e in ents):
             a, b, sums = ops.stats_norm_finalize(ents, spatial, mode, groups=groups, weight=weight, bias=bias)
             for t, sm in zip(parts, sums):
@@ -441,7 +483,8 @@
             return self._conv(cache, [x], b.prefix + ".conv", b.cout, 3, upsample=True, out_size=up_size)
         raise ValueError(b.kind)
 
-    def _stem(self, feat: Optional[torch.Tensor], cache: dict, proj0: Optional[torch.Tensor] = None) -> torch.Tensor:
+    def _stem(self, feat: Optional[torch.Tensor], cache: dict, proj0: Optional[torch.Tensor] = None,
+              proj0_stats: Optional[PendingTileStats] = None) -> torch.Tensor:
         cfg, ops = self.cfg, self.ops
         spatial = (proj0 if proj0 is not None else feat)[0].numel()
         x = feat
@@ -457,6 +500,8 @@
             else:
                 hid = cfg.projector_hidden
                 x = proj0 if proj0 is not None else self._conv(cache, [x], q + "0", hid, 1)
+                if proj0 is not None and proj0_stats is not None:
+                    self._remember(cache, x, proj0_stats, proj0_stats.slot)
                 pro = self._norm(cache, [x], spatial, 1, groups=32, weight=self.p[q + "1.weight"], bias=self.p[q + "1.bias"])
                 x = self._conv(cache, [x], q + "3", hid, 3, pro=pro, act=ACT_SILU, bound=self._norm_bound(q + "1", spatial * (hid // 32)))
                 pro = self._norm(cache, [x], spatial, 1, groups=32, weight=self.p[q + "4.weight"], bias=self.p[q + "4.bias"])
@@ -471,7 +516,8 @@
         return self._conv(cache, [h], "unet.out.2", self.cfg.out_channels, 3, pro=pro, affine_key="unet.out.0", act=ACT_LEAKY,
                           bound=self._norm_bound("unet.out.0", h[0].numel()))
 
-    def forward(self, feat: Optional[torch.Tensor], taps: Optional[dict] = None, proj0: Optional[torch.Tensor] = None) -> torch.Tensor:
+    def forward(self, feat: Optional[torch.Tensor], taps: Optional[dict] = None, proj0: Optional[torch.Tensor] = None,
+                proj0_stats: Optional[PendingTileStats] = None) -> torch.Tensor:
         cache: dict = {}
         only = set(taps) if taps else None
 
@@ -481,7 +527,7 @@
 
         plan = self.plan
         hs: List[torch.Tensor] = []
-        h = self._stem(feat, cache, proj0)
+        h = self._stem(feat, cache, proj0, proj0_stats)
         hs.append(h)
         tap("unet.input_blocks.0", h)
         for seq in plan.input_blocks[1:]:
@@ -553,7 +599,8 @@
             raise _lib.PixieHipError(self.lib.pixie_last_error().decode())
         return n
 
-    def forward(self, feat: Optional[torch.Tensor], proj0: Optional[torch.Tensor] = None, workspace: Optional[torch.Tensor] = None) -> torch.Tensor:
+    def forward(self, feat: Optional[torch.Tensor], proj0: Optional[torch.Tensor] = None, workspace: Optional[torch.Tensor] = None,
+                proj0_stats: Optional[PendingTileStats] = None) -> torch.Tensor:
         src = proj0 if proj0 is not None else feat
         d, h, w = (int(v) for v in src.shape[1:])
         out = torch.empty((self.cfg.out_channels, d, h, w), device=self.device, dtype=torch.float32)
@@ -562,6 +609,10 @@
             workspace = torch.empty(nbytes, device=self.device, dtype=torch.uint8)
         elif workspace.dtype != torch.uint8 or workspace.device != self.device or workspace.numel() < nbytes or not workspace.is_contiguous():
             raise ValueError(f"workspace must be a contiguous uint8 tensor of >= {nbytes} bytes on {self.device}")
+        if proj0 is not None and proj0_stats is not None:
+            check(self.lib.pixie_unet_forward_proj0(self._h, _ptr(proj0), _ptr(proj0_stats.stats), _ptr(proj0_stats.slot), d, h, w, _ptr(out),
+                                                    _ptr(workspace), nbytes, _lib.current_stream_ptr()), "pixie_unet_forward_proj0")
+            return out
         check(self.lib.pixie_unet_forward(self._h, _ptr(feat), _ptr(proj0), d, h, w, _ptr(out), _ptr(workspace), nbytes,
                                           _lib.current_stream_ptr()), "pixie_unet_forward")
         return out
@@ -591,6 +642,7 @@
         self.conv_precision = DEFAULT_PRECISION
         self.use_graph = os.environ.get("PIXIE_UNET_GRAPH", "1") == "1"
         self._graphs: dict = {}
+        self.graph_captures = 0
         self._plist = None
 
     @staticmethod
@@ -637,10 +689,11 @@
         elif self.executor != "python":
             raise ValueError(f"unknown executor {self.executor!r} (PIXIE_UNET_EXECUTOR is 'c' or 'python')")
 
-    def _forward_one(self, x: Optional[torch.Tensor], taps: Optional[dict] = None, proj0: Optional[torch.Tensor] = None) -> torch.Tensor:
+    def _forward_one(self, x: Optional[torch.Tensor], taps: Optional[dict] = None, proj0: Optional[torch.Tensor] = None,
+                     proj0_stats: Optional[PendingTileStats] = None) -> torch.Tensor:
         if self.executor == "c" and taps is None:
-            return self._handle.forward(x, proj0)
-        return self._runner.forward(x, taps, proj0)
+            return self._handle.forward(x, proj0, proj0_stats=proj0_stats)
+        return self._runner.forward(x, taps, proj0, proj0_stats)
 
     def _apply(self, fn, *args, **kwargs):
         self._plist = None
@@ -656,11 +709,12 @@
         self._plist = None
         return super().load_state_dict(state_dict, strict=strict, assign=assign)
 
-    def _forward_graphed(self, x: Optional[torch.Tensor], proj0: Optional[torch.Tensor] = None) -> torch.Tensor:
+    def _forward_graphed(self, x: Optional[torch.Tensor], proj0: Optional[torch.Tensor] = None,
+                         proj0_stats: Optional[PendingTileStats] = None) -> torch.Tensor:
         src = proj0 if proj0 is not None else x
-        base = (tuple(src.shape), tuple(src.stride()), src.dtype, proj0 is not None, self.executor, self.conv_precision, src.device.index,
+        base = (tuple(src.shape), tuple(src.stride()), src.dtype, proj0 is not None, _addr(proj0_stats.stats) if proj0_stats else None, self.executor, self.conv_precision, src.device.index,
                 tuple((id(p), p.data_ptr(), p._version) for p in self._param_list()))
-        run = (lambda t: self._forward_one(None, proj0=t)) if proj0 is not None else (lambda t: self._forward_one(t))
+        run = (lambda t: self._forward_one(None, proj0=t, proj0_stats=proj0_stats)) if proj0 is not None else (lambda t: self._forward_one(t))
         if self._graphs.get("base") != base:
             self._graphs = {"base": base, "first_ptr": None}
         ent = self._graphs.get(src.data_ptr()) or self._graphs.get("copy")
@@ -669,8 +723,8 @@
             if self._graphs["first_ptr"] is None:
                 self._graphs["first_ptr"] = src.data_ptr()
                 return out
-            in_place = (proj0 is None and self._graphs["first_ptr"] == src.data_ptr() and "copy" not in self._graphs
-                        and os.environ.get("PIXIE_UNET_GRAPH_INPLACE", "1") == "1")
+            in_place = ((proj0 is None or proj0_stats is not None) and self._graphs["first_ptr"] == src.data_ptr() and "copy" not in self._graphs
+                        and (proj0_stats is not None or os.environ.get("PIXIE_UNET_GRAPH_INPLACE", "1") == "1"))
             try:
                 static_in = src if in_place else src.clone()
                 side = torch.cuda.Stream(src.device)
@@ -686,6 +740,7 @@
                               RuntimeWarning)
                 self.use_graph = False
                 return out
+            self.graph_captures += 1
             if in_place:
                 ent = self._graphs[src.data_ptr()] = (graph, None, static_out)
             else:
@@ -770,6 +825,74 @@
     return _SIDE_STREAMS[key]
 
 
+class Conv0Shared:
+
+    def __init__(self, ops: HipOps, cont_network, shape, hid: int):
+        c, d, h, w = shape
+        dev = ops.device
+        self.key = (id(cont_network), dev, tuple(shape))
+        self.outs = [torch.empty((hid, d, h, w), device=dev, dtype=torch.float32) for _ in range(2)]
+        nfl = ops.conv0_stats_floats(d * h * w, hid)
+        self.stats = [torch.empty(nfl, device=dev, dtype=torch.float32) for _ in range(2)]
+        self.slots = torch.zeros(4, device=dev, dtype=torch.int32)
+        self.pending = [PendingTileStats(self.stats[i], self.slots[1 + i:2 + i], hid) for i in range(2)]
+
+    def launch(self, ops: HipOps, feat: torch.Tensor, packed) -> None:
+        self.slots.zero_()
+        ops.tensor_amax(feat, self.slots[0:1])
+        ops.projector_conv0_f32(feat, packed, self.outs[0].shape[0], self.slots[0:1], outs=self.outs, stats=self.stats,
+                                out_amax=[p.slot for p in self.pending])
+
+
+def _shared_conv0_ok(seg_network, cont_network, feat_grid: torch.Tensor) -> bool:
+    if os.environ.get("PIXIE_SHARED_CONV0", "1") == "0" or not feat_grid.is_cuda or feat_grid.dim() != 5:
+        return False
+    a, b = seg_network.cfg, cont_network.cfg
+    return (a.projector_hidden is not None and b.projector_hidden == a.projector_hidden and a.feature_channels == b.feature_channels
+            and a.feature_channels % 16 == 0 and feat_grid.shape[1] == a.feature_channels and a.grid_size == b.grid_size
+            and seg_network.conv_precision == "f16x3" and cont_network.conv_precision == "f16x3"
+            and next(seg_network.parameters()).device == feat_grid.device == next(cont_network.parameters()).device
+            and _lib.load().pixie_conv_cout_padded(a.projector_hidden) * 2 == 256)
+
+
+def _predict_shared_conv0(seg_network, cont_network, feat_grid: torch.Tensor, dual_stream: bool):
+    dev = feat_grid.device
+    nets = (seg_network, cont_network)
+    for net in nets:
+        net._prepare(dev)
+    ops = seg_network._runner.ops
+    x = feat_grid.detach().to(torch.float32).contiguous()
+    shared = seg_network.__dict__.get("_conv0_shared")
+    if shared is None or shared.key != (id(cont_network), dev, tuple(x.shape[1:])):
+        seg_network.__dict__["_conv0_shared"] = None
+        shared = seg_network.__dict__["_conv0_shared"] = Conv0Shared(ops, cont_network, tuple(x.shape[1:]), seg_network.cfg.projector_hidden)
+    q = "projector.net.0"
+    packed = [(net._runner._w16(q), net._runner._b(q)) for net in nets]
+
+    def fwd(net, i):
+        if net.use_graph:
+            return net._forward_graphed(None, shared.outs[i], shared.pending[i])
+        return net._forward_one(None, proj0=shared.outs[i], proj0_stats=shared.pending[i])
+
+    cur = torch.cuda.current_stream()
+    seg_logits, cont_pred = [], []
+    for n in range(x.shape[0]):
+        shared.launch(ops, x[n], packed)
+        if dual_stream:
+            s1, s2 = _side_streams(dev)
+            s1.wait_stream(cur); s2.wait_stream(cur)
+            with torch.cuda.stream(s1):
+                a = fwd(seg_network, 0)
+            with torch.cuda.stream(s2):
+                b = fwd(cont_network, 1)
+            cur.wait_stream(s1); cur.wait_stream(s2)
+            a.record_stream(cur); b.record_stream(cur)
+        else:
+            a, b = fwd(seg_network, 0), fwd(cont_network, 1)
+        seg_logits.append(a); cont_pred.append(b)
+    return torch.stack(seg_logits), torch.stack(cont_pred)
+
+
 @torch.no_grad()
 def predict_material_field(seg_network: SegmentationUNet, cont_network: RegressionUNet, feat_grid: torch.Tensor,
                            dual_stream: Optional[bool] = None):
@@ -778,7 +901,10 @@
             return predict_material_field(seg_network, cont_network, feat_grid, dual_stream)
     if dual_stream is None:
         dual_stream = _dual_stream_default(seg_network, cont_network, int(feat_grid[0, 0].numel()))
-    if dual_stream and feat_grid.is_cuda:
+    if _shared_conv0_ok(seg_network, cont_network, feat_grid):
+        with torch.cuda.device(feat_grid.device):
+            seg_logits, cont_pred = _predict_shared_conv0(seg_network, cont_network, feat_grid, bool(dual_stream))
+    elif dual_stream and feat_grid.is_cuda:
         cur = torch.cuda.current_stream()
         s1, s2 = _side_streams(feat_grid.device)
         s1.wait_stream(cur); s2.wait_stream(cur)
```

Measured after the change: 24.81 million voxels/s, median of 2. Within noise of the previous version (+0.0%).
